# defuse/zebra

Measured on AMD Instinct MI355X. Metric: Sapling Groth16 proofs verified/sec (batch 64k) at 1/2/4/8 MI355X, higher is better.
Workload: dtype u32

## Files before the change

zebra_amd/csrc/gen_fq29.py:

```python
#!/usr/bin/env python3
import sys

P = 0x1a0111ea397fe69a4b1ba7b6434bacd764774b84f38512bf6730d2a0f6b0f6241eabfffeb153ffffb9feffffffffaaab
D = 14
W = 29
MASK = (1 << W) - 1
P29 = [(P >> (W * i)) & MASK for i in range(D)]
PINV = (-pow(P, -1, 1 << W)) % (1 << W)
_q = [((2 * P) >> (W * i)) & MASK for i in range(D)]
P2B = [_q[i] + ((1 << W) if i < D - 1 else 0) - (1 if i > 0 else 0) for i in range(D)]
assert sum(b << (W * i) for i, b in enumerate(P2B)) == 2 * P and all(b >= MASK for b in P2B[:D - 1])
assert P2B[D - 1] >= (P >> (W * (D - 1)))


KP_MAX = 12


def borrowed(k):
    q = [((k * P) >> (W * i)) & MASK for i in range(D)]
    if k == 0:
        return q
    b = [q[i] + ((1 << W) if i < D - 1 else 0) - (1 if i > 0 else 0) for i in range(D)]
    assert sum(x << (W * i) for i, x in enumerate(b)) == k * P and all(x >= MASK for x in b[:D - 1])
    if k >= 2:
        assert ((k - 1) * P) >> (W * (D - 1)) <= b[D - 1], k
    return b


def split(dst, src):
    out = []
    for L in range(D):
        b = W * L
        w, o = b >> 5, b & 31
        if o + W <= 32:
            e = "%s[%d]" % (src, w) if o == 0 else "(%s[%d] >> %d)" % (src, w, o)
            if o + W < 32:
                e = "%s & FQ29_MASK" % e
        elif w + 1 < 12:
            e = "zg_alignbit(%s[%d], %s[%d], %d) & FQ29_MASK" % (src, w + 1, src, w, o)
        else:
            e = "%s[%d] >> %d" % (src, w, o)
            out.append("  %s[%d] = %s;" % (dst, L, e))
            out.append("  zg_opaque(%s[%d]);  // narrow top digit: see gen_mont29" % (dst, L))
            continue
        out.append("  %s[%d] = %s;" % (dst, L, e))
    return out


def terms(a, b, k, step=1):
    return [(a, i, b, k - i) for i in range(D) if 0 <= k - i < D]


def sq_terms(a, a2, k):
    t = [(a2, i, a, k - i) for i in range(D) if i < k - i < D]
    if k % 2 == 0 and k // 2 < D:
        t.append((a, k // 2, a, k // 2))
    return t


def redc(chains, canon=True):
    out = []
    for (r, a, _) in chains:
        out.append("  uint32_t %s_m[14], %s_u[14];" % (a, a))
        out.append("  uint64_t %s = 0;" % a)
    for k in range(2 * D - 1):
        cols = [(r, a, f(k)) for (r, a, f) in chains]
        n = max(len(t) for _, _, t in cols)
        for q in range(n):
            for (r, a, t) in cols:
                if q < len(t):
                    x, i, y, j = t[q]
                    out.append("  %s += (uint64_t)%s[%d] * %s[%d];" % (a, x, i, y, j))
        for j in range(D):
            if j < k and k - j < D:
                for (r, a, _) in cols:
                    out.append("  %s += (uint64_t)%s_m[%d] * 0x%08xu;" % (a, a, j, P29[k - j]))
        for (r, a, _) in cols:
            if k < D - 1:
                out.append("  %s_m[%d] = ((uint32_t)%s * 0x%08xu) & FQ29_MASK;" % (a, k, a, PINV))
            elif k == D - 1:
                out.append("  %s_m[%d] = ((uint32_t)%s * 0x%08xu) & 127u;" % (a, k, a, PINV))
                out.append("  zg_opaque(%s_m[%d]);" % (a, k))
        for (r, a, _) in cols:
            if k <= D - 1:
                out.append("  %s += (uint64_t)%s_m[%d] * 0x%08xu;" % (a, a, k, P29[0]))
            if k >= D - 1:
                out.append("  %s_u[%d] = (uint32_t)%s & FQ29_MASK;" % (a, k - (D - 1), a))
            out.append("  %s >>= 29;" % a)
    for (r, a, _) in chains:
        for w in range(12):
            b = 7 + 32 * w
            L, o = b // W, b % W
            parts = ["(%s_u[%d] >> %d)" % (a, L, o) if o else "%s_u[%d]" % (a, L),
                     "(%s_u[%d] << %d)" % (a, L + 1, W - o)]
            if o + 32 > 2 * W:
                parts.append("(%s_u[%d] << %d)" % (a, L + 2, 2 * W - o))
            tgt = "%s_t[%d]" % (a, w) if canon else "%s[%d]" % (r, w)
            if w == 0 and canon:
                out.append("  uint32_t %s_t[12];" % a)
            out.append("  %s = %s;" % (tgt, " | ".join(parts)))
        if canon:
            out.append("  fq29_canon(%s, %s_t);" % (r, a))
    return out


def redc_full(chains):
    out = []
    for (r, a, _) in chains:
        out.append("  uint32_t %s_m[14];" % a)
        out.append("  uint64_t %s = 0;" % a)
    for k in range(2 * D - 1):
        cols = [(r, a, f(k)) for (r, a, f) in chains]
        n = max(len(t) for _, _, t in cols)
        for q in range(n):
            for (r, a, t) in cols:
                if q < len(t):
                    x, i, y, j = t[q]
                    out.append("  %s += (uint64_t)%s[%d] * %s[%d];" % (a, x, i, y, j))
        for j in range(D):
            if j < k and k - j < D:
                for (r, a, _) in cols:
                    out.append("  %s += (uint64_t)%s_m[%d] * 0x%08xu;" % (a, a, j, P29[k - j]))
        for (r, a, _) in cols:
            if k < D:
                out.append("  %s_m[%d] = ((uint32_t)%s * 0x%08xu) & FQ29_MASK;" % (a, k, a, PINV))
                out.append("  %s += (uint64_t)%s_m[%d] * 0x%08xu;" % (a, a, k, P29[0]))
            else:
                out.append("  %s[%d] = (uint32_t)%s & FQ29_MASK;" % (r, k - D, a))
            out.append("  %s >>= 29;" % a)
    for (r, a, _) in chains:
        out.append("  %s[13] = (uint32_t)%s;" % (r, a))
    return out


def gen_mont29(name, M, NW, mname, doc_bound):
    Dm = -(-32 * NW // W)
    last = 32 * NW - W * (Dm - 1)
    Md = [(M >> (W * i)) & MASK for i in range(Dm)]
    pinv = (-pow(M, -1, 1 << W)) % (1 << W)
    assert 2 * Dm * (1 << 58) < 1 << 64
    out = ["  uint32_t A[%d], B[%d], m[%d], u[%d], t[%d];" % (Dm, Dm, Dm, Dm + 1, NW), "  uint64_t acc = 0;"]
    for L in range(Dm):
        b_ = W * L
        w, o_ = b_ >> 5, b_ & 31
        for (X, src) in (("A", "a"), ("B", "b")):
            if o_ + W <= 32:
                e = "%s[%d]" % (src, w) if o_ == 0 else "(%s[%d] >> %d)" % (src, w, o_)
                if o_ + W < 32:
                    e += " & FQ29_MASK"
            elif w + 1 < NW:
                e = "zg_alignbit(%s[%d], %s[%d], %d) & FQ29_MASK" % (src, w + 1, src, w, o_)
            else:
                e = "%s[%d] >> %d" % (src, w, o_)
            out.append("  %s[%d] = %s;" % (X, L, e))
    out.append("  zg_opaque(A[%d]); zg_opaque(B[%d]);" % (Dm - 1, Dm - 1))
    for k in range(2 * Dm - 1):
        for i in range(Dm):
            if 0 <= k - i < Dm:
                out.append("  acc += (uint64_t)A[%d] * B[%d];" % (i, k - i))
        for j in range(Dm):
            if j < k and k - j < Dm:
                out.append("  acc += (uint64_t)m[%d] * 0x%08xu;" % (j, Md[k - j]))
        if k < Dm - 1:
            out.append("  m[%d] = ((uint32_t)acc * 0x%08xu) & FQ29_MASK;" % (k, pinv))
        elif k == Dm - 1:
            out.append("  m[%d] = ((uint32_t)acc * 0x%08xu) & 0x%08xu;" % (k, pinv, (1 << last) - 1))
            out.append("  zg_opaque(m[%d]);" % k)
        if k <= Dm - 1:
            out.append("  acc += (uint64_t)m[%d] * 0x%08xu;" % (k, Md[0]))
        if k >= Dm - 1:
            out.append("  u[%d] = (uint32_t)acc & FQ29_MASK;" % (k - (Dm - 1)))
        out.append("  acc >>= 29;")
    out.append("  u[%d] = (uint32_t)acc;  // u = t 2^%d < 2M 2^%d needs a digit more" % (Dm, last, last))
    for w in range(NW):
        b_ = last + 32 * w
        L, o_ = b_ // W, b_ % W
        parts = ["(u[%d] >> %d)" % (L, o_) if o_ else "u[%d]" % L]
        if L + 1 <= Dm:
            parts.append("(u[%d] << %d)" % (L + 1, W - o_))
        if o_ + 32 > 2 * W and L + 2 <= Dm:
            parts.append("(u[%d] << %d)" % (L + 2, 2 * W - o_))
        out.append("  t[%d] = %s;" % (w, " | ".join(parts)))
    out += ["#if defined(__HIP_DEVICE_COMPILE__)",
            "  uint32_t pm[%d];" % NW,
            "#pragma unroll",
            "  for (int i = 0; i < %d; i++) pm[i] = %s[i];" % (NW, mname),
            "  mp_reduce_once<%d>(r, t, pm);" % NW,
            "#else",
            "  uint32_t d[%d];" % NW, "  uint64_t bo = 0;",
            "  for (int i = 0; i < %d; i++) {" % NW,
            "    const uint64_t x = (uint64_t)t[i] - %s[i] - bo;" % mname,
            "    d[i] = (uint32_t)x;", "    bo = (x >> 63) & 1;", "  }",
            "  for (int i = 0; i < %d; i++) r[i] = bo ? t[i] : d[i];" % NW,
            "#endif"]
    return fn(name, "uint32_t* r, const uint32_t* a, const uint32_t* b", out,
              ["r = a b 2^-%d mod %s in 29-bit digits (%d digits, mixed radix: %d x 29 + %d): %s" % (
                  32 * NW, mname, Dm, Dm - 1, last, doc_bound)])


def fn(name, args, body, doc):
    return ["// " + d for d in doc] + ["ZG_INL void %s(%s) {" % (name, args)] + body + ["}", ""]


def main():
    o = ["// GENERATED by zebra_amd/csrc/gen_fq29.py -- do not edit.", "#pragma once", "namespace zg {", ""]
    o.append("static constexpr uint32_t FQ29_MASK = 0x%08xu;" % MASK)
    o.append("static constexpr uint32_t FQ_2P_B29[14] = {%s};  // 2p, digits 0..12 >= 2^29 - 1" %
             ", ".join("0x%08xu" % x for x in P2B))
    o.append("")
    o += ["ZG_INL uint32_t zg_alignbit(uint32_t hi, uint32_t lo, int s) {",
          "#if defined(__HIP_DEVICE_COMPILE__)",
          "  return __builtin_amdgcn_alignbit(hi, lo, s);",
          "#else",
          "  return (uint32_t)((((uint64_t)hi << 32) | lo) >> s);",
          "#endif",
          "}", ""]
    o += ["// an optimisation barrier: the compiler forgets what it knows about x's range (no instruction)",
          "ZG_INL void zg_opaque(uint32_t& x) {",
          "#if defined(__HIP_DEVICE_COMPILE__)",
          '  asm volatile("" : "+v"(x));',
          "#else",
          "  (void)x;",
          "#endif",
          "}", ""]
    o += ["// r = t >= p ? t - p : t  (t < 2p)",
          "ZG_INL void fq29_canon(uint32_t* r, const uint32_t* t) {",
          "#if defined(__HIP_DEVICE_COMPILE__)",
          "  uint32_t pm[12];",
          "#pragma unroll",
          "  for (int i = 0; i < 12; i++) pm[i] = FQ_P[i];",
          "  mp_reduce_once<12>(r, t, pm);",
          "#else",
          "  uint32_t d[12];",
          "  uint64_t bo = 0;",
          "  for (int i = 0; i < 12; i++) {",
          "    const uint64_t x = (uint64_t)t[i] - FQ_P[i] - bo;",
          "    d[i] = (uint32_t)x;",
          "    bo = (x >> 63) & 1;",
          "  }",
          "  for (int i = 0; i < 12; i++) r[i] = bo ? t[i] : d[i];",
          "#endif",
          "}", ""]

    body = ["  uint32_t A[14], B[14];"] + split("A", "a") + split("B", "b")
    body += redc([("r", "acc", lambda k: terms("A", "B", k))])
    o += fn("fq29_mul", "uint32_t* r, const uint32_t* a, const uint32_t* b", body,
            ["r = a b 2^-384 mod p; a b < 2^384 p (e.g. a < 4p, b < 2p) -> r < p.",
             "Column bound: 14 a*b + 14 m*p terms < 2^58 each."])
    body = ["  uint32_t A[14], A2[14];"] + split("A", "a") + ["  A2[%d] = A[%d] << 1;" % (i, i) for i in range(D)]
    body += redc([("r", "acc", lambda k: sq_terms("A", "A2", k))])
    o += fn("fq29_sqr", "uint32_t* r, const uint32_t* a", body,
            ["r = a^2 2^-384 mod p for a < 2p (a^2 < 2^384 p) -> r < p: 105 digit products, the",
             "off-diagonal ones once with a doubled operand (< 2^59: 7 + 14 terms per column, fine)."])
    body = ["  uint32_t X0[14], X1[14], Y0[14], Y1[14], N1[14];"] + split("X0", "x0") + split("X1", "x1") + \
        split("Y0", "y0") + split("Y1", "y1") + ["  N1[%d] = 0x%08xu - Y1[%d];" % (i, P2B[i], i) for i in range(D)]
    body += redc([("c0", "a0", lambda k: terms("X0", "Y0", k) + terms("X1", "N1", k)),
                  ("c1", "a1", lambda k: terms("X0", "Y1", k) + terms("X1", "Y0", k))])
    o += fn("f2_mul29", "uint32_t* c0, uint32_t* c1, const uint32_t* x0, const uint32_t* x1, const uint32_t* y0, "
            "const uint32_t* y1", body,
            ["Fq2 product, schoolbook in 29-bit digits with two reductions:",
             "  c0 = REDC(x0 y0 + x1 (2p - y1)),  c1 = REDC(x0 y1 + x1 y0)",
             "x lazy (< 2p per coefficient), y canonical: c0's sum < 2p p + 2p 2p = 6p^2 < 2^384 p, so both",
             "results are < p after the conditional subtraction (the contract of f2_mul_kind). Column bound",
             "for c0: 14 terms < 2^58, 14 terms < 2^59 (2p - y1 digits < 2^30), 14 m*p terms: < 2^64."])
    body = ["  uint32_t X0[14], X1[14], S[14];"] + split("X0", "x0") + split("X1", "x1") + split("S", "s")
    body += redc([("c0", "a0", lambda k: terms("X0", "S", k)), ("c1", "a1", lambda k: terms("X1", "S", k))])
    o += fn("f2_mul_fq29", "uint32_t* c0, uint32_t* c1, const uint32_t* x0, const uint32_t* x1, const uint32_t* s",
            body, ["(x0 s, x1 s) for x lazy (< 2p), s canonical -> canonical"])
    body = ["  uint32_t X0[14], X1[14], D[14], S[14], T[14];"] + split("X0", "x0") + split("X1", "x1") + \
        split("D", "dif") + ["  S[%d] = X0[%d] + X1[%d];\n  T[%d] = X1[%d] << 1;" % (i, i, i, i, i) for i in range(D)]
    body += redc([("c0", "a0", lambda k: terms("S", "D", k)), ("c1", "a1", lambda k: terms("X0", "T", k))])
    o += fn("f2_sqr29", "uint32_t* c0, uint32_t* c1, const uint32_t* x0, const uint32_t* x1, const uint32_t* dif",
            body, ["x^2 for canonical x given dif = x0 - x1 mod p: c0 = (x0 + x1) dif, c1 = x0 (2 x1). The sum and",
                   "the doubled digits are formed digit-wise (< 2^30). Column bound: 14 terms < 2^59 + 14 m*p."])
    RP = 2 ** (D * W)
    kin = (2 ** (2 * D * W - 384)) % P
    kout = (2 ** 384) % P
    o.append("static constexpr uint32_t FQ29D_KIN[14] = {%s};  // 2^428 mod p: R -> R' = 2^406" %
             ", ".join("0x%08xu" % ((kin >> (W * i)) & MASK) for i in range(D)))
    o.append("static constexpr uint32_t FQ29D_KOUT[14] = {%s};  // 2^384 mod p: R' -> R" %
             ", ".join("0x%08xu" % ((kout >> (W * i)) & MASK) for i in range(D)))
    o.append("")
    body = redc_full([("r", "acc", lambda k: terms("a", "b", k))])
    o += fn("fq29d_mul", "uint32_t* r, const uint32_t* a, const uint32_t* b", body,
            ["r = a b 2^-406 mod p in digits: a, b < 2p (normalized digits) -> r < 2p (normalized).",
             "r may alias neither a nor b."])
    body = ["  uint32_t A2[14];"] + ["  A2[%d] = a[%d] << 1;" % (i, i) for i in range(D)]
    body += redc_full([("r", "acc", lambda k: sq_terms("a", "A2", k))])
    o += fn("fq29d_sqr", "uint32_t* r, const uint32_t* a", body,
            ["r = a^2 2^-406 mod p in digits (a < 2p) -> r < 2p; r may not alias a."])
    body = ["  uint32_t A[14];"] + split("A", "a")
    body += redc_full([("r", "acc", lambda k: terms("A", "FQ29D_KIN", k))])
    o += fn("fq29d_from_mont", "uint32_t* r, const uint32_t* a",
            body, ["12-word a R (any a < 2^384) -> 14-digit a R' (< 2p)"])
    body = ["  uint32_t u[14], t[12];"] + redc_full([("u", "acc", lambda k: terms("a", "FQ29D_KOUT", k))])
    for w in range(12):
        b_ = 32 * w
        L, o_ = b_ // W, b_ % W
        parts = ["(u[%d] >> %d)" % (L, o_) if o_ else "u[%d]" % L, "(u[%d] << %d)" % (L + 1, W - o_)]
        if o_ + 32 > 2 * W:
            parts.append("(u[%d] << %d)" % (L + 2, 2 * W - o_))
        body.append("  t[%d] = %s;" % (w, " | ".join(parts)))
    body.append("  fq29_canon(r, t);")
    o += fn("fq29d_to_mont", "uint32_t* r, const uint32_t* a", body,
            ["14-digit a R' (< 2p) -> canonical 12-word a R"])

    body = redc_full([("r0", "a0", lambda k: terms("a", "b", k)), ("r1", "a1", lambda k: terms("c", "d", k))])
    o += fn("fq29d_mul2", "uint32_t* r0, uint32_t* r1, const uint32_t* a, const uint32_t* b, const uint32_t* c, "
            "const uint32_t* d", body,
            ["r0 = a b 2^-406, r1 = c d 2^-406 mod p in digits, the two chains interleaved (an Fq2 square as",
             "(x0 + x1)(x0 - x1), x0 (2 x1); an Fq2 times an Fq). Digit bounds: max(a) max(b) < 3.5 2^58, same",
             "for c d (one operand may hold unnormalized digits < 2^30). Outputs normalized, < a b / 2^406 + p."])
    body = redc_full([("c0", "a0", lambda k: terms("x0", "y0", k) + terms("x1", "n1", k)),
                      ("c1", "a1", lambda k: terms("x0", "y1", k) + terms("x1", "y0", k))])
    o += fn("f2d_mul29", "uint32_t* c0, uint32_t* c1, const uint32_t* x0, const uint32_t* x1, const uint32_t* y0, "
            "const uint32_t* y1, const uint32_t* n1", body,
            ["Fq2 product in digits, schoolbook with two reductions (the MAC structure of f2_mul29):",
             "  c0 = REDC'(x0 y0 + x1 n1),  c1 = REDC'(x0 y1 + x1 y0),  n1 = k p - y1 digit-wise (>= 0).",
             "x, y normalized (digits < 2^29), n1 digits < 2^30: 14 (2^58 + 2^59) + 14 2^58 < 2^64."])
    body = ["  uint32_t t[12];"]
    for w in range(12):
        b_ = 32 * w
        L, o_ = b_ // W, b_ % W
        parts = ["(u[%d] >> %d)" % (L, o_) if o_ else "u[%d]" % L, "(u[%d] << %d)" % (L + 1, W - o_)]
        if o_ + 32 > 2 * W:
            parts.append("(u[%d] << %d)" % (L + 2, 2 * W - o_))
        body.append("  t[%d] = %s;" % (w, " | ".join(parts)))
    body.append("  fq29_canon(r, t);")
    o += fn("fq29d_pack", "uint32_t* r, const uint32_t* u", body,
            ["14 normalized digits of a value < 2p -> its canonical 12 words (the repack and conditional",
             "subtraction that close fq29_mul)"])
    for (nm, sh, doc) in (("fq29d_split", 0, "12 words -> 14 digits of the same value"),
                          ("fq29d_split22", 22, "12 words a -> 14 digits of 2^22 a (a R -> a R' = 2^406, "
                                                "unreduced: < 2^22 p for canonical a)")):
        body = []
        for L in range(D):
            s_ = W * L - sh
            if s_ < 0:
                body.append("  d[%d] = (a[0] << %d) & FQ29_MASK;" % (L, -s_))
                continue
            w, o_ = s_ >> 5, s_ & 31
            if o_ + W <= 32:
                e = "a[%d]" % w if o_ == 0 else "(a[%d] >> %d)" % (w, o_)
                if o_ + W < 32:
                    e += " & FQ29_MASK"
            elif w + 1 < 12:
                e = "zg_alignbit(a[%d], a[%d], %d) & FQ29_MASK" % (w + 1, w, o_)
            else:
                e = "a[%d] >> %d" % (w, o_)
            body.append("  d[%d] = %s;" % (L, e))
            if w + 1 >= 12 and o_ + W > 32:
                body.append("  zg_opaque(d[%d]);  // narrow top digit: see gen_mont29" % L)
        o += fn(nm, "uint32_t* d, const uint32_t* a", body, [doc])
    pinv22 = PINV & ((1 << 22) - 1)
    assert (P * pinv22 + 1) % (1 << 22) == 0
    body = ["  uint32_t u[14], t[12];", "  uint32_t m = (a[0] * 0x%08xu) & 0x3fffffu;" % pinv22, "  zg_opaque(m);",
            "  uint64_t acc = 0;"]
    for k in range(D):
        body.append("  acc += a[%d];" % k)
        body.append("  acc += (uint64_t)m * 0x%08xu;" % P29[k])
        body.append("  u[%d] = (uint32_t)acc%s;" % (k, " & FQ29_MASK" if k < D - 1 else ""))
        if k < D - 1:
            body.append("  acc >>= 29;")
    for w in range(12):
        b_ = 22 + 32 * w
        L, o_ = b_ // W, b_ % W
        parts = ["(u[%d] >> %d)" % (L, o_) if o_ else "u[%d]" % L, "(u[%d] << %d)" % (L + 1, W - o_)]
        if o_ + 32 > 2 * W and L + 2 < D:
            parts.append("(u[%d] << %d)" % (L + 2, 2 * W - o_))
        body.append("  t[%d] = %s;" % (w, " | ".join(parts)))
    body.append("  fq29_canon(r, t);")
    o += fn("fq29d_red22", "uint32_t* r, const uint32_t* a", body,
            ["14-digit a R' (normalized, any value < 2^22 p) -> canonical 12-word a R: (a + m p) / 2^22 with",
             "m = -a / p mod 2^22, < 2p before the conditional subtraction"])

    R_BLS = 0x73eda753299d7d483339d80809a1d80553bda402fffe5bfeffffffff00000001
    P_BN = 0x30644e72e131a029b85045b68181585d97816a916871ca8d3c208c16d87cfd47
    o += gen_mont29("fr29_mul", R_BLS, 8, "FR_R", "a, b < r -> r' < r")
    o += gen_mont29("bq29_mul", P_BN, 8, "BQ_P", "a, b < p -> r < p")

    o.append("#define ZG_KP_MAX %d" % KP_MAX)
    o.append("// k p (12 words) and k p with borrowed 29-bit digits (digits 0..12 >= 2^29 - 1, top digit")
    o.append("// >= the top digit of any y <= (k - 1) p), k = 0..%d" % KP_MAX)
    o.append("static constexpr uint32_t FQ_KP[%d][12] = {%s};" % (KP_MAX + 1, ", ".join(
        "{%s}" % ", ".join("0x%08xu" % ((k * P >> (32 * i)) & 0xffffffff) for i in range(12)) for k in range(KP_MAX + 1))))
    o.append("static constexpr uint32_t FQ_KP_B29[%d][14] = {%s};" % (KP_MAX + 1, ", ".join(
        "{%s}" % ", ".join("0x%08xu" % x for x in borrowed(k)) for k in range(KP_MAX + 1))))
    o.append("")
    body = ["  uint32_t X0[14], X1[14], Y0[14], Y1[14], N1[14];"] + split("X0", "x0") + split("X1", "x1") + \
        split("Y0", "y0") + split("Y1", "y1") + ["  N1[%d] = off[%d] - Y1[%d];" % (i, i, i) for i in range(D)]
    body += redc([("c0", "a0", lambda k: terms("X0", "Y0", k) + terms("X1", "N1", k)),
                  ("c1", "a1", lambda k: terms("X0", "Y1", k) + terms("X1", "Y0", k))], canon=False)
    o += fn("f2_mul29_raw", "uint32_t* c0, uint32_t* c1, const uint32_t* x0, const uint32_t* x1, const uint32_t* y0, "
            "const uint32_t* y1, const uint32_t* off", body,
            ["f2_mul29 with y1 <= (k - 1) p and off = FQ_KP_B29[k]: c0 = REDC(x0 y0 + x1 (k p - y1)),",
             "c1 = REDC(x0 y1 + x1 y0), unreduced (< S / 2^384 + p). x, y < 2^384 (digits < 2^29)."])
    body = ["  uint32_t X0[14], X1[14], S[14];"] + split("X0", "x0") + split("X1", "x1") + split("S", "s")
    body += redc([("c0", "a0", lambda k: terms("X0", "S", k)), ("c1", "a1", lambda k: terms("X1", "S", k))],
                 canon=False)
    o += fn("f2_mul_fq29_raw", "uint32_t* c0, uint32_t* c1, const uint32_t* x0, const uint32_t* x1, const uint32_t* s",
            body, ["(x0 s, x1 s), unreduced"])
    body = ["  uint32_t X0[14], X1[14], D[14], S[14], T[14];"] + split("X0", "x0") + split("X1", "x1") + \
        split("D", "dif") + ["  S[%d] = X0[%d] + X1[%d];\n  T[%d] = X1[%d] << 1;" % (i, i, i, i, i) for i in range(D)]
    body += redc([("c0", "a0", lambda k: terms("S", "D", k)), ("c1", "a1", lambda k: terms("X0", "T", k))],
                 canon=False)
    o += fn("f2_sqr29_raw", "uint32_t* c0, uint32_t* c1, const uint32_t* x0, const uint32_t* x1, const uint32_t* dif",
            body, ["x^2 with dif = x0 - x1 + k p (any x < 2^384): c0 = (x0 + x1) dif, c1 = x0 (2 x1), unreduced"])
    o.append("}  // namespace zg")
    sys.stdout.write("\n".join(o) + "\n")


if __name__ == "__main__":
    main()
```

zebra_amd/csrc/zg_decode.h:

```cpp
#pragma once
#include "zg_batch.h"

namespace zg {

#ifndef ZG_DECODE_FQD
#define ZG_DECODE_FQD 1
#endif
#if ZG_DECODE_FQD
#define ZG_DEC_SUBGROUP g1_in_subgroup_d
#ifndef ZG_DEC_GLV
#define ZG_DEC_GLV g1_glv_mul_d
#endif
#else
#define ZG_DEC_SUBGROUP g1_in_subgroup
#define ZG_DEC_GLV g1_glv_mul
#endif

#if defined(ZG_TU_DECODE_SQRT)
#ifndef ZG_DECODE_SQRT_WPE
#define ZG_DECODE_SQRT_WPE ZG_DECODE_WPE
#endif
__global__ void __launch_bounds__(64, ZG_DECODE_SQRT_WPE) k_decode_sqrt(BatchBufs b) {
  const int role = blockIdx.x & 1;
  const int i = (blockIdx.x >> 1) * 64 + (threadIdx.x & 63);
  if (blockIdx.x == 0 && threadIdx.x < 2) b.bfail[threadIdx.x] = 0;
  if (i >= b.npad) return;
  G1A p;
  p.inf = true;
  if (i < b.n && g1_decompress(b.proofs + (size_t)i * 192 + (role == 0 ? 0 : 144), &p, false) != DEC_OK)
    p.inf = true;
  b.ptAC[(size_t)role * b.npad + i] = p;
}
#else

#if ZG_DECODE_FQD
struct GlvTabLds {
  uint32_t* base;
  __device__ __forceinline__ void put(int e, int c, const FqD& v) const {
#pragma unroll
    for (int d = 0; d < 14; d++) base[((e * 2 + c) * 14 + d) * 64] = v.d[d];
  }
  __device__ __forceinline__ FqD get(int e, int c) const {
    FqD v;
#pragma unroll
    for (int d = 0; d < 14; d++) v.d[d] = base[((e * 2 + c) * 14 + d) * 64];
    return v;
  }
};
__global__ void __launch_bounds__(64, ZG_DECODE_WPE) k_decode_glv_lds(BatchBufs b) {
  __shared__ uint32_t lds_tab[8 * 2 * 14 * 64];
  const int i = blockIdx.x * 64 + (threadIdx.x & 63);
  if (i >= b.npad) return;
  const G1A p = b.ptAC[i];
  G1A o;
  o.inf = true;
  if (!p.inf) {
    uint64_t ra, rb;
    batch_scalar_ab(b.r + (size_t)i * 16, &ra, &rb);
    const GlvTabLds tab{lds_tab + (threadIdx.x & 63)};
    G1J j;
    g1_glv_mul_w2_t(&j, &p, ra, rb, tab);
    o = jac_to_aff(j);
  }
  b.ptA[i] = o;
}
#endif

template <int JOB>
__global__ void __launch_bounds__(64, ZG_DECODE_WPE) k_decode_points(BatchBufs b, int cglv) {
  const int G = (b.npad + 63) / 64, nglv = cglv ? 2 * G : G;
  const int blk = JOB == -2 ? nglv + (int)blockIdx.x : JOB <= 0 ? (int)blockIdx.x : JOB == 1 ? nglv + (int)blockIdx.x
                                                                                     : nglv + 2 * G + (int)blockIdx.x;
  const int job = JOB >= 0 ? JOB : blk < nglv ? 0 : blk < nglv + 2 * G ? 1 : 2;
  const int role = job == 0 ? (blk < G ? 0 : 1) : job == 2 ? 2 : ((blk - nglv) & 1);
  const int grp = job == 0 ? (blk < G ? blk : blk - G) : job == 2 ? blk - nglv - 2 * G : (blk - nglv) >> 1;
  const int i = grp * 64 + (threadIdx.x & 63);
  if (i >= b.npad) return;
  if (job == 2) {
    G2A q;
    q.inf = true;
    bool ok = false;
    if (i < b.n) ok = g2_decompress(b.proofs + (size_t)i * 192 + 48, &q, false) == DEC_OK;
    b.ptB[i] = q;
    b.okbits[3 * i + 2] = ok;
    return;
  }
  const G1A p = b.ptAC[(size_t)role * b.npad + i];
  const bool ok = !p.inf;
  if (job == 1) {
    b.okbits[3 * i + role] = ok && ZG_DEC_SUBGROUP(p);
    return;
  }
  uint64_t ra = 0, rb = 0;
  if (ok) batch_scalar_ab(b.r + (size_t)i * 16, &ra, &rb);
  if (role == 1) {
    const int kind = i < b.n ? b.kinds[i] : 0;
    const G1J o = ok ? ZG_DEC_GLV(p, ra, rb) : jac_infinity<Fq>();
    for (int k = 0; k < ZG_NKINDS; k++) b.ctree[((size_t)b.npad + i) * ZG_NKINDS + k] = k == kind ? o : jac_infinity<Fq>();
    return;
  }
  G1A o;
  o.inf = true;
  if (ok) o = jac_to_aff(ZG_DEC_GLV(p, ra, rb));
  b.ptA[i] = o;
}

__global__ void __launch_bounds__(64) k_decode_finish(BatchBufs b) {
  const int i = blockIdx.x * 64 + (threadIdx.x & 63);
  if (i >= b.npad) return;
  const bool live = i < b.n;
  const int leaf = b.npad + i;
  const int kind = live ? b.kinds[i] : 0;
  uint8_t st = ST_PENDING;
  int k = 0, kk = 0;
  const uint8_t* in = b.inputs + (size_t)i * 288;
  if (live) {
    k = b.ninputs ? b.ninputs[i] : KIND_NINPUTS[kind];
    kk = k < ZG_MAX_INPUTS ? k : ZG_MAX_INPUTS;
    const bool ok = b.okbits[3 * i] && b.okbits[3 * i + 1] && b.okbits[3 * i + 2];
    bool canon = true;
#pragma unroll
    for (int j = 0; j < ZG_MAX_INPUTS; j++)
      if (j < kk) canon = canon && fp_lt_modulus<FrM>(fr_limbs_from_le(in + 32 * j));
    if (!canon)
      st = ST_INPUT_NONCANONICAL;
    else if (!ok)
      st = ST_DECODE_INVALID;
    else if (k + 1 != b.vks[kind].ic_len)
      st = ST_MALFORMED_VK;
    b.status[i] = st;
  }
  const bool pend = live && st == ST_PENDING;
  if (!pend) b.ptA[i].inf = true;
  if (!pend)
    for (int kd = 0; kd < ZG_NKINDS; kd++) b.ctree[(size_t)leaf * ZG_NKINDS + kd] = jac_infinity<Fq>();
  b.ptB[i].inf = !(live && (st == ST_PENDING || st == ST_MALFORMED_VK));
  for (int kd = 0; kd < ZG_NKINDS; kd++) {
    Fr* s = b.stree + (leaf * ZG_NKINDS + kd) * ZG_MAX_IC;
    for (int m = 0; m < ZG_MAX_IC; m++) s[m] = fp_zero<FrM>();
  }
  if (pend) {
    uint64_t ra, rb;
    batch_scalar_ab(b.r + (size_t)i * 16, &ra, &rb);
    const Fr rf = batch_scalar_fr(ra, rb);
    Fr* s = b.stree + (leaf * ZG_NKINDS + kind) * ZG_MAX_IC;
    s[0] = rf;
#pragma unroll
    for (int j = 0; j < ZG_MAX_INPUTS; j++)
      if (j < kk) s[1 + j] = fr_mul(rf, fr_to_mont(fr_limbs_from_le(in + 32 * j)));
  }
}

#endif

}
```

zebra_amd/csrc/zg_fq29_gen.h:

```cpp
#pragma once
namespace zg {

static constexpr uint32_t FQ29_MASK = 0x1fffffffu;
static constexpr uint32_t FQ_2P_B29[14] = {0x3fff5556u, 0x3feffffeu, 0x29ffffdbu, 0x2ffffac4u, 0x3ec483d4u, 0x32a0f6afu, 0x35fb3985u, 0x213ce143u, 0x2ec8ee96u, 0x2434baccu, 0x258dd3dau, 0x25ff9a68u, 0x20223d46u, 0x00000019u};

ZG_INL uint32_t zg_alignbit(uint32_t hi, uint32_t lo, int s) {
#if defined(__HIP_DEVICE_COMPILE__)
  return __builtin_amdgcn_alignbit(hi, lo, s);
#else
  return (uint32_t)((((uint64_t)hi << 32) | lo) >> s);
#endif
}

ZG_INL void zg_opaque(uint32_t& x) {
#if defined(__HIP_DEVICE_COMPILE__)
  asm volatile("" : "+v"(x));
#else
  (void)x;
#endif
}

ZG_INL void fq29_canon(uint32_t* r, const uint32_t* t) {
#if defined(__HIP_DEVICE_COMPILE__)
  uint32_t pm[12];
// ... 4821 lines not shown
  acc += (uint64_t)acc_m[0] * 0x0afd9cc3u;
  acc += (uint64_t)acc_m[1] * 0x09507b58u;
  acc += (uint64_t)acc_m[2] * 0x0f6241eau;
  acc += (uint64_t)acc_m[3] * 0x17fffd62u;
  acc += (uint64_t)acc_m[4] * 0x14ffffeeu;
  acc += (uint64_t)acc_m[5] * 0x0ff7ffffu;
  acc_m[6] = ((uint32_t)acc * 0x1ffcfffdu) & FQ29_MASK;
  acc += (uint64_t)acc_m[6] * 0x1fffaaabu;
  acc >>= 29;
  acc += (uint64_t)A2[0] * a[7];
  acc += (uint64_t)A2[1] * a[6];
  acc += (uint64_t)A2[2] * a[5];
  acc += (uint64_t)A2[3] * a[4];
  acc += (uint64_t)acc_m[0] * 0x109e70a2u;
  acc += (uint64_t)acc_m[1] * 0x0afd9cc3u;
  acc += (uint64_t)acc_m[2] * 0x09507b58u;
  acc += (uint64_t)acc_m[3] * 0x0f6241eau;
  acc += (uint64_t)acc_m[4] * 0x17fffd62u;
  acc += (uint64_t)acc_m[5] * 0x14ffffeeu;
  acc += (uint64_t)acc_m[6] * 0x0ff7ffffu;
  acc_m[7] = ((uint32_t)acc * 0x1ffcfffdu) & FQ29_MASK;
  acc += (uint64_t)acc_m[7] * 0x1fffaaabu;
  acc >>= 29;
  acc += (uint64_t)A2[0] * a[8];
  acc += (uint64_t)A2[1] * a[7];
  acc += (uint64_t)A2[2] * a[6];
  acc += (uint64_t)A2[3] * a[5];
  acc += (uint64_t)a[4] * a[4];
  acc += (uint64_t)acc_m[0] * 0x1764774bu;
  acc += (uint64_t)acc_m[1] * 0x109e70a2u;
  acc += (uint64_t)acc_m[2] * 0x0afd9cc3u;
  acc += (uint64_t)acc_m[3] * 0x09507b58u;
  acc += (uint64_t)acc_m[4] * 0x0f6241eau;
  acc += (uint64_t)acc_m[5] * 0x17fffd62u;
  acc += (uint64_t)acc_m[6] * 0x14ffffeeu;
  acc += (uint64_t)acc_m[7] * 0x0ff7ffffu;
  acc_m[8] = ((uint32_t)acc * 0x1ffcfffdu) & FQ29_MASK;
  acc += (uint64_t)acc_m[8] * 0x1fffaaabu;
  acc >>= 29;
  acc += (uint64_t)A2[0] * a[9];
  acc += (uint64_t)A2[1] * a[8];
  acc += (uint64_t)A2[2] * a[7];
  acc += (uint64_t)A2[3] * a[6];
  acc += (uint64_t)A2[4] * a[5];
  acc += (uint64_t)acc_m[0] * 0x121a5d66u;
  acc += (uint64_t)acc_m[1] * 0x1764774bu;
  acc += (uint64_t)acc_m[2] * 0x109e70a2u;
  acc += (uint64_t)acc_m[3] * 0x0afd9cc3u;
  acc += (uint64_t)acc_m[4] * 0x09507b58u;
  acc += (uint64_t)acc_m[5] * 0x0f6241eau;
  acc += (uint64_t)acc_m[6] * 0x17fffd62u;
  acc += (uint64_t)acc_m[7] * 0x14ffffeeu;
  acc += (uint64_t)acc_m[8] * 0x0ff7ffffu;
  acc_m[9] = ((uint32_t)acc * 0x1ffcfffdu) & FQ29_MASK;
  acc += (uint64_t)acc_m[9] * 0x1fffaaabu;
  acc >>= 29;
  acc += (uint64_t)A2[0] * a[10];
  acc += (uint64_t)A2[1] * a[9];
  acc += (uint64_t)A2[2] * a[8];
  acc += (uint64_t)A2[3] * a[7];
  acc += (uint64_t)A2[4] * a[6];
  acc += (uint64_t)a[5] * a[5];
  acc += (uint64_t)acc_m[0] * 0x12c6e9edu;
  acc += (uint64_t)acc_m[1] * 0x121a5d66u;
  acc += (uint64_t)acc_m[2] * 0x1764774bu;
  acc += (uint64_t)acc_m[3] * 0x109e70a2u;
  acc += (uint64_t)acc_m[4] * 0x0afd9cc3u;
  acc += (uint64_t)acc_m[5] * 0x09507b58u;
  acc += (uint64_t)acc_m[6] * 0x0f6241eau;
  acc += (uint64_t)acc_m[7] * 0x17fffd62u;
  acc += (uint64_t)acc_m[8] * 0x14ffffeeu;
  acc += (uint64_t)acc_m[9] * 0x0ff7ffffu;
  acc_m[10] = ((uint32_t)acc * 0x1ffcfffdu) & FQ29_MASK;
  acc += (uint64_t)acc_m[10] * 0x1fffaaabu;
  acc >>= 29;
  acc += (uint64_t)A2[0] * a[11];
  acc += (uint64_t)A2[1] * a[10];
  acc += (uint64_t)A2[2] * a[9];
  acc += (uint64_t)A2[3] * a[8];
  acc += (uint64_t)A2[4] * a[7];
  acc += (uint64_t)A2[5] * a[6];
  acc += (uint64_t)acc_m[0] * 0x12ffcd34u;
  acc += (uint64_t)acc_m[1] * 0x12c6e9edu;
  acc += (uint64_t)acc_m[2] * 0x121a5d66u;
  acc += (uint64_t)acc_m[3] * 0x1764774bu;
  acc += (uint64_t)acc_m[4] * 0x109e70a2u;
  acc += (uint64_t)acc_m[5] * 0x0afd9cc3u;
  acc += (uint64_t)acc_m[6] * 0x09507b58u;
  acc += (uint64_t)acc_m[7] * 0x0f6241eau;
  acc += (uint64_t)acc_m[8] * 0x17fffd62u;
  acc += (uint64_t)acc_m[9] * 0x14ffffeeu;
  acc += (uint64_t)acc_m[10] * 0x0ff7ffffu;
  acc_m[11] = ((uint32_t)acc * 0x1ffcfffdu) & FQ29_MASK;
  acc += (uint64_t)acc_m[11] * 0x1fffaaabu;
  acc >>= 29;
  acc += (uint64_t)A2[0] * a[12];
  acc += (uint64_t)A2[1] * a[11];
  acc += (uint64_t)A2[2] * a[10];
  acc += (uint64_t)A2[3] * a[9];
  acc += (uint64_t)A2[4] * a[8];
  acc += (uint64_t)A2[5] * a[7];
  acc += (uint64_t)a[6] * a[6];
  acc += (uint64_t)acc_m[0] * 0x00111ea3u;
  acc += (uint64_t)acc_m[1] * 0x12ffcd34u;
  acc += (uint64_t)acc_m[2] * 0x12c6e9edu;
  acc += (uint64_t)acc_m[3] * 0x121a5d66u;
  acc += (uint64_t)acc_m[4] * 0x1764774bu;
  acc += (uint64_t)acc_m[5] * 0x109e70a2u;
  acc += (uint64_t)acc_m[6] * 0x0afd9cc3u;
  acc += (uint64_t)acc_m[7] * 0x09507b58u;
  acc += (uint64_t)acc_m[8] * 0x0f6241eau;
  acc += (uint64_t)acc_m[9] * 0x17fffd62u;
  acc += (uint64_t)acc_m[10] * 0x14ffffeeu;
  acc += (uint64_t)acc_m[11] * 0x0ff7ffffu;
  acc_m[12] = ((uint32_t)acc * 0x1ffcfffdu) & FQ29_MASK;
  acc += (uint64_t)acc_m[12] * 0x1fffaaabu;
  acc >>= 29;
  acc += (uint64_t)A2[0] * a[13];
  acc += (uint64_t)A2[1] * a[12];
  acc += (uint64_t)A2[2] * a[11];
  acc += (uint64_t)A2[3] * a[10];
  acc += (uint64_t)A2[4] * a[9];
  acc += (uint64_t)A2[5] * a[8];
  acc += (uint64_t)A2[6] * a[7];
  acc += (uint64_t)acc_m[0] * 0x0000000du;
  acc += (uint64_t)acc_m[1] * 0x00111ea3u;
  acc += (uint64_t)acc_m[2] * 0x12ffcd34u;
  acc += (uint64_t)acc_m[3] * 0x12c6e9edu;
  acc += (uint64_t)acc_m[4] * 0x121a5d66u;
  acc += (uint64_t)acc_m[5] * 0x1764774bu;
  acc += (uint64_t)acc_m[6] * 0x109e70a2u;
  acc += (uint64_t)acc_m[7] * 0x0afd9cc3u;
  acc += (uint64_t)acc_m[8] * 0x09507b58u;
  acc += (uint64_t)acc_m[9] * 0x0f6241eau;
  acc += (uint64_t)acc_m[10] * 0x17fffd62u;
  acc += (uint64_t)acc_m[11] * 0x14ffffeeu;
  acc += (uint64_t)acc_m[12] * 0x0ff7ffffu;
  acc_m[13] = ((uint32_t)acc * 0x1ffcfffdu) & FQ29_MASK;
  acc += (uint64_t)acc_m[13] * 0x1fffaaabu;
  acc >>= 29;
  acc += (uint64_t)A2[1] * a[13];
  acc += (uint64_t)A2[2] * a[12];
  acc += (uint64_t)A2[3] * a[11];
  acc += (uint64_t)A2[4] * a[10];
  acc += (uint64_t)A2[5] * a[9];
  acc += (uint64_t)A2[6] * a[8];
  acc += (uint64_t)a[7] * a[7];
  acc += (uint64_t)acc_m[1] * 0x0000000du;
  acc += (uint64_t)acc_m[2] * 0x00111ea3u;
  acc += (uint64_t)acc_m[3] * 0x12ffcd34u;
  acc += (uint64_t)acc_m[4] * 0x12c6e9edu;
  acc += (uint64_t)acc_m[5] * 0x121a5d66u;
  acc += (uint64_t)acc_m[6] * 0x1764774bu;
  acc += (uint64_t)acc_m[7] * 0x109e70a2u;
  acc += (uint64_t)acc_m[8] * 0x0afd9cc3u;
  acc += (uint64_t)acc_m[9] * 0x09507b58u;
  acc += (uint64_t)acc_m[10] * 0x0f6241eau;
  acc += (uint64_t)acc_m[11] * 0x17fffd62u;
  acc += (uint64_t)acc_m[12] * 0x14ffffeeu;
  acc += (uint64_t)acc_m[13] * 0x0ff7ffffu;
  r[0] = (uint32_t)acc & FQ29_MASK;
  acc >>= 29;
  acc += (uint64_t)A2[2] * a[13];
  acc += (uint64_t)A2[3] * a[12];
  acc += (uint64_t)A2[4] * a[11];
  acc += (uint64_t)A2[5] * a[10];
  acc += (uint64_t)A2[6] * a[9];
  acc += (uint64_t)A2[7] * a[8];
  acc += (uint64_t)acc_m[2] * 0x0000000du;
  acc += (uint64_t)acc_m[3] * 0x00111ea3u;
  acc += (uint64_t)acc_m[4] * 0x12ffcd34u;
  acc += (uint64_t)acc_m[5] * 0x12c6e9edu;
  acc += (uint64_t)acc_m[6] * 0x121a5d66u;
  acc += (uint64_t)acc_m[7] * 0x1764774bu;
  acc += (uint64_t)acc_m[8] * 0x109e70a2u;
  acc += (uint64_t)acc_m[9] * 0x0afd9cc3u;
  acc += (uint64_t)acc_m[10] * 0x09507b58u;
  acc += (uint64_t)acc_m[11] * 0x0f6241eau;
  acc += (uint64_t)acc_m[12] * 0x17fffd62u;
  acc += (uint64_t)acc_m[13] * 0x14ffffeeu;
  r[1] = (uint32_t)acc & FQ29_MASK;
  acc >>= 29;
  acc += (uint64_t)A2[3] * a[13];
  acc += (uint64_t)A2[4] * a[12];
  acc += (uint64_t)A2[5] * a[11];
  acc += (uint64_t)A2[6] * a[10];
  acc += (uint64_t)A2[7] * a[9];
  acc += (uint64_t)a[8] * a[8];
  acc += (uint64_t)acc_m[3] * 0x0000000du;
  acc += (uint64_t)acc_m[4] * 0x00111ea3u;
  acc += (uint64_t)acc_m[5] * 0x12ffcd34u;
  acc += (uint64_t)acc_m[6] * 0x12c6e9edu;
  acc += (uint64_t)acc_m[7] * 0x121a5d66u;
  acc += (uint64_t)acc_m[8] * 0x1764774bu;
  acc += (uint64_t)acc_m[9] * 0x109e70a2u;
  acc += (uint64_t)acc_m[10] * 0x0afd9cc3u;
  acc += (uint64_t)acc_m[11] * 0x09507b58u;
  acc += (uint64_t)acc_m[12] * 0x0f6241eau;
  acc += (uint64_t)acc_m[13] * 0x17fffd62u;
  r[2] = (uint32_t)acc & FQ29_MASK;
  acc >>= 29;
  acc += (uint64_t)A2[4] * a[13];
  acc += (uint64_t)A2[5] * a[12];
  acc += (uint64_t)A2[6] * a[11];
  acc += (uint64_t)A2[7] * a[10];
  acc += (uint64_t)A2[8] * a[9];
  acc += (uint64_t)acc_m[4] * 0x0000000du;
  acc += (uint64_t)acc_m[5] * 0x00111ea3u;
  acc += (uint64_t)acc_m[6] * 0x12ffcd34u;
  acc += (uint64_t)acc_m[7] * 0x12c6e9edu;
  acc += (uint64_t)acc_m[8] * 0x121a5d66u;
  acc += (uint64_t)acc_m[9] * 0x1764774bu;
  acc += (uint64_t)acc_m[10] * 0x109e70a2u;
  acc += (uint64_t)acc_m[11] * 0x0afd9cc3u;
  acc += (uint64_t)acc_m[12] * 0x09507b58u;
  acc += (uint64_t)acc_m[13] * 0x0f6241eau;
  r[3] = (uint32_t)acc & FQ29_MASK;
  acc >>= 29;
  acc += (uint64_t)A2[5] * a[13];
  acc += (uint64_t)A2[6] * a[12];
  acc += (uint64_t)A2[7] * a[11];
  acc += (uint64_t)A2[8] * a[10];
  acc += (uint64_t)a[9] * a[9];
  acc += (uint64_t)acc_m[5] * 0x0000000du;
  acc += (uint64_t)acc_m[6] * 0x00111ea3u;
  acc += (uint64_t)acc_m[7] * 0x12ffcd34u;
  acc += (uint64_t)acc_m[8] * 0x12c6e9edu;
  acc += (uint64_t)acc_m[9] * 0x121a5d66u;
  acc += (uint64_t)acc_m[10] * 0x1764774bu;
  acc += (uint64_t)acc_m[11] * 0x109e70a2u;
  acc += (uint64_t)acc_m[12] * 0x0afd9cc3u;
  acc += (uint64_t)acc_m[13] * 0x09507b58u;
  r[4] = (uint32_t)acc & FQ29_MASK;
  acc >>= 29;
  acc += (uint64_t)A2[6] * a[13];
  acc += (uint64_t)A2[7] * a[12];
  acc += (uint64_t)A2[8] * a[11];
  acc += (uint64_t)A2[9] * a[10];
  acc += (uint64_t)acc_m[6] * 0x0000000du;
  acc += (uint64_t)acc_m[7] * 0x00111ea3u;
  acc += (uint64_t)acc_m[8] * 0x12ffcd34u;
  acc += (uint64_t)acc_m[9] * 0x12c6e9edu;
  acc += (uint64_t)acc_m[10] * 0x121a5d66u;
  acc += (uint64_t)acc_m[11] * 0x1764774bu;
  acc += (uint64_t)acc_m[12] * 0x109e70a2u;
  acc += (uint64_t)acc_m[13] * 0x0afd9cc3u;
  r[5] = (uint32_t)acc & FQ29_MASK;
  acc >>= 29;
  acc += (uint64_t)A2[7] * a[13];
  acc += (uint64_t)A2[8] * a[12];
  acc += (uint64_t)A2[9] * a[11];
  acc += (uint64_t)a[10] * a[10];
  acc += (uint64_t)acc_m[7] * 0x0000000du;
  acc += (uint64_t)acc_m[8] * 0x00111ea3u;
  acc += (uint64_t)acc_m[9] * 0x12ffcd34u;
  acc += (uint64_t)acc_m[10] * 0x12c6e9edu;
  acc += (uint64_t)acc_m[11] * 0x121a5d66u;
  acc += (uint64_t)acc_m[12] * 0x1764774bu;
  acc += (uint64_t)acc_m[13] * 0x109e70a2u;
  r[6] = (uint32_t)acc & FQ29_MASK;
  acc >>= 29;
  acc += (uint64_t)A2[8] * a[13];
  acc += (uint64_t)A2[9] * a[12];
  acc += (uint64_t)A2[10] * a[11];
  acc += (uint64_t)acc_m[8] * 0x0000000du;
  acc += (uint64_t)acc_m[9] * 0x00111ea3u;
  acc += (uint64_t)acc_m[10] * 0x12ffcd34u;
  acc += (uint64_t)acc_m[11] * 0x12c6e9edu;
  acc += (uint64_t)acc_m[12] * 0x121a5d66u;
  acc += (uint64_t)acc_m[13] * 0x1764774bu;
  r[7] = (uint32_t)acc & FQ29_MASK;
  acc >>= 29;
  acc += (uint64_t)A2[9] * a[13];
  acc += (uint64_t)A2[10] * a[12];
  acc += (uint64_t)a[11] * a[11];
  acc += (uint64_t)acc_m[9] * 0x0000000du;
  acc += (uint64_t)acc_m[10] * 0x00111ea3u;
  acc += (uint64_t)acc_m[11] * 0x12ffcd34u;
  acc += (uint64_t)acc_m[12] * 0x12c6e9edu;
  acc += (uint64_t)acc_m[13] * 0x121a5d66u;
  r[8] = (uint32_t)acc & FQ29_MASK;
  acc >>= 29;
  acc += (uint64_t)A2[10] * a[13];
  acc += (uint64_t)A2[11] * a[12];
  acc += (uint64_t)acc_m[10] * 0x0000000du;
  acc += (uint64_t)acc_m[11] * 0x00111ea3u;
  acc += (uint64_t)acc_m[12] * 0x12ffcd34u;
  acc += (uint64_t)acc_m[13] * 0x12c6e9edu;
  r[9] = (uint32_t)acc & FQ29_MASK;
  acc >>= 29;
  acc += (uint64_t)A2[11] * a[13];
  acc += (uint64_t)a[12] * a[12];
  acc += (uint64_t)acc_m[11] * 0x0000000du;
  acc += (uint64_t)acc_m[12] * 0x00111ea3u;
  acc += (uint64_t)acc_m[13] * 0x12ffcd34u;
  r[10] = (uint32_t)acc & FQ29_MASK;
  acc >>= 29;
  acc += (uint64_t)A2[12] * a[13];
  acc += (uint64_t)acc_m[12] * 0x0000000du;
  acc += (uint64_t)acc_m[13] * 0x00111ea3u;
  r[11] = (uint32_t)acc & FQ29_MASK;
  acc >>= 29;
  acc += (uint64_t)a[13] * a[13];
  acc += (uint64_t)acc_m[13] * 0x0000000du;
  r[12] = (uint32_t)acc & FQ29_MASK;
  acc >>= 29;
  r[13] = (uint32_t)acc;
}

ZG_INL void fq29d_from_mont(uint32_t* r, const uint32_t* a) {
  uint32_t A[14];
  A[0] = a[0] & FQ29_MASK;
  A[1] = zg_alignbit(a[1], a[0], 29) & FQ29_MASK;
  A[2] = zg_alignbit(a[2], a[1], 26) & FQ29_MASK;
  A[3] = zg_alignbit(a[3], a[2], 23) & FQ29_MASK;
  A[4] = zg_alignbit(a[4], a[3], 20) & FQ29_MASK;
  A[5] = zg_alignbit(a[5], a[4], 17) & FQ29_MASK;
  A[6] = zg_alignbit(a[6], a[5], 14) & FQ29_MASK;
  A[7] = zg_alignbit(a[7], a[6], 11) & FQ29_MASK;
  A[8] = zg_alignbit(a[8], a[7], 8) & FQ29_MASK;
  A[9] = zg_alignbit(a[9], a[8], 5) & FQ29_MASK;
  A[10] = (a[9] >> 2) & FQ29_MASK;
  A[11] = zg_alignbit(a[10], a[9], 31) & FQ29_MASK;
  A[12] = zg_alignbit(a[11], a[10], 28) & FQ29_MASK;
  A[13] = a[11] >> 25;
  zg_opaque(A[13]);
  uint32_t acc_m[14];
  uint64_t acc = 0;
  acc += (uint64_t)A[0] * FQ29D_KIN[0];
  acc_m[0] = ((uint32_t)acc * 0x1ffcfffdu) & FQ29_MASK;
  acc += (uint64_t)acc_m[0] * 0x1fffaaabu;
  acc >>= 29;
  acc += (uint64_t)A[0] * FQ29D_KIN[1];
  acc += (uint64_t)A[1] * FQ29D_KIN[0];
  acc += (uint64_t)acc_m[0] * 0x0ff7ffffu;
  acc_m[1] = ((uint32_t)acc * 0x1ffcfffdu) & FQ29_MASK;
  acc += (uint64_t)acc_m[1] * 0x1fffaaabu;
  acc >>= 29;
  acc += (uint64_t)A[0] * FQ29D_KIN[2];
  acc += (uint64_t)A[1] * FQ29D_KIN[1];
  acc += (uint64_t)A[2] * FQ29D_KIN[0];
  acc += (uint64_t)acc_m[0] * 0x14ffffeeu;
  acc += (uint64_t)acc_m[1] * 0x0ff7ffffu;
  acc_m[2] = ((uint32_t)acc * 0x1ffcfffdu) & FQ29_MASK;
  acc += (uint64_t)acc_m[2] * 0x1fffaaabu;
  acc >>= 29;
  acc += (uint64_t)A[0] * FQ29D_KIN[3];
  acc += (uint64_t)A[1] * FQ29D_KIN[2];
  acc += (uint64_t)A[2] * FQ29D_KIN[1];
  acc += (uint64_t)A[3] * FQ29D_KIN[0];
  acc += (uint64_t)acc_m[0] * 0x17fffd62u;
  acc += (uint64_t)acc_m[1] * 0x14ffffeeu;
  acc += (uint64_t)acc_m[2] * 0x0ff7ffffu;
  acc_m[3] = ((uint32_t)acc * 0x1ffcfffdu) & FQ29_MASK;
  acc += (uint64_t)acc_m[3] * 0x1fffaaabu;
  acc >>= 29;
  acc += (uint64_t)A[0] * FQ29D_KIN[4];
  acc += (uint64_t)A[1] * FQ29D_KIN[3];
  acc += (uint64_t)A[2] * FQ29D_KIN[2];
  acc += (uint64_t)A[3] * FQ29D_KIN[1];
  acc += (uint64_t)A[4] * FQ29D_KIN[0];
  acc += (uint64_t)acc_m[0] * 0x0f6241eau;
  acc += (uint64_t)acc_m[1] * 0x17fffd62u;
  acc += (uint64_t)acc_m[2] * 0x14ffffeeu;
  acc += (uint64_t)acc_m[3] * 0x0ff7ffffu;
  acc_m[4] = ((uint32_t)acc * 0x1ffcfffdu) & FQ29_MASK;
  acc += (uint64_t)acc_m[4] * 0x1fffaaabu;
  acc >>= 29;
  acc += (uint64_t)A[0] * FQ29D_KIN[5];
  acc += (uint64_t)A[1] * FQ29D_KIN[4];
  acc += (uint64_t)A[2] * FQ29D_KIN[3];
  acc += (uint64_t)A[3] * FQ29D_KIN[2];
  acc += (uint64_t)A[4] * FQ29D_KIN[1];
  acc += (uint64_t)A[5] * FQ29D_KIN[0];
  acc += (uint64_t)acc_m[0] * 0x09507b58u;
  acc += (uint64_t)acc_m[1] * 0x0f6241eau;
  acc += (uint64_t)acc_m[2] * 0x17fffd62u;
  acc += (uint64_t)acc_m[3] * 0x14ffffeeu;
  acc += (uint64_t)acc_m[4] * 0x0ff7ffffu;
  acc_m[5] = ((uint32_t)acc * 0x1ffcfffdu) & FQ29_MASK;
  acc += (uint64_t)acc_m[5] * 0x1fffaaabu;
  acc >>= 29;
  acc += (uint64_t)A[0] * FQ29D_KIN[6];
  acc += (uint64_t)A[1] * FQ29D_KIN[5];
  acc += (uint64_t)A[2] * FQ29D_KIN[4];
  acc += (uint64_t)A[3] * FQ29D_KIN[3];
  acc += (uint64_t)A[4] * FQ29D_KIN[2];
  acc += (uint64_t)A[5] * FQ29D_KIN[1];
  acc += (uint64_t)A[6] * FQ29D_KIN[0];
  acc += (uint64_t)acc_m[0] * 0x0afd9cc3u;
  acc += (uint64_t)acc_m[1] * 0x09507b58u;
  acc += (uint64_t)acc_m[2] * 0x0f6241eau;
  acc += (uint64_t)acc_m[3] * 0x17fffd62u;
  acc += (uint64_t)acc_m[4] * 0x14ffffeeu;
  acc += (uint64_t)acc_m[5] * 0x0ff7ffffu;
  acc_m[6] = ((uint32_t)acc * 0x1ffcfffdu) & FQ29_MASK;
  acc += (uint64_t)acc_m[6] * 0x1fffaaabu;
  acc >>= 29;
  acc += (uint64_t)A[0] * FQ29D_KIN[7];
  acc += (uint64_t)A[1] * FQ29D_KIN[6];
  acc += (uint64_t)A[2] * FQ29D_KIN[5];
  acc += (uint64_t)A[3] * FQ29D_KIN[4];
  acc += (uint64_t)A[4] * FQ29D_KIN[3];
  acc += (uint64_t)A[5] * FQ29D_KIN[2];
  acc += (uint64_t)A[6] * FQ29D_KIN[1];
  acc += (uint64_t)A[7] * FQ29D_KIN[0];
  acc += (uint64_t)acc_m[0] * 0x109e70a2u;
  acc += (uint64_t)acc_m[1] * 0x0afd9cc3u;
  acc += (uint64_t)acc_m[2] * 0x09507b58u;
  acc += (uint64_t)acc_m[3] * 0x0f6241eau;
  acc += (uint64_t)acc_m[4] * 0x17fffd62u;
  acc += (uint64_t)acc_m[5] * 0x14ffffeeu;
  acc += (uint64_t)acc_m[6] * 0x0ff7ffffu;
  acc_m[7] = ((uint32_t)acc * 0x1ffcfffdu) & FQ29_MASK;
  acc += (uint64_t)acc_m[7] * 0x1fffaaabu;
  acc >>= 29;
  acc += (uint64_t)A[0] * FQ29D_KIN[8];
  acc += (uint64_t)A[1] * FQ29D_KIN[7];
  acc += (uint64_t)A[2] * FQ29D_KIN[6];
  acc += (uint64_t)A[3] * FQ29D_KIN[5];
  acc += (uint64_t)A[4] * FQ29D_KIN[4];
  acc += (uint64_t)A[5] * FQ29D_KIN[3];
  acc += (uint64_t)A[6] * FQ29D_KIN[2];
  acc += (uint64_t)A[7] * FQ29D_KIN[1];
  acc += (uint64_t)A[8] * FQ29D_KIN[0];
  acc += (uint64_t)acc_m[0] * 0x1764774bu;
  acc += (uint64_t)acc_m[1] * 0x109e70a2u;
  acc += (uint64_t)acc_m[2] * 0x0afd9cc3u;
  acc += (uint64_t)acc_m[3] * 0x09507b58u;
  acc += (uint64_t)acc_m[4] * 0x0f6241eau;
  acc += (uint64_t)acc_m[5] * 0x17fffd62u;
  acc += (uint64_t)acc_m[6] * 0x14ffffeeu;
  acc += (uint64_t)acc_m[7] * 0x0ff7ffffu;
  acc_m[8] = ((uint32_t)acc * 0x1ffcfffdu) & FQ29_MASK;
  acc += (uint64_t)acc_m[8] * 0x1fffaaabu;
  acc >>= 29;
  acc += (uint64_t)A[0] * FQ29D_KIN[9];
  acc += (uint64_t)A[1] * FQ29D_KIN[8];
  acc += (uint64_t)A[2] * FQ29D_KIN[7];
  acc += (uint64_t)A[3] * FQ29D_KIN[6];
  acc += (uint64_t)A[4] * FQ29D_KIN[5];
  acc += (uint64_t)A[5] * FQ29D_KIN[4];
  acc += (uint64_t)A[6] * FQ29D_KIN[3];
  acc += (uint64_t)A[7] * FQ29D_KIN[2];
  acc += (uint64_t)A[8] * FQ29D_KIN[1];
  acc += (uint64_t)A[9] * FQ29D_KIN[0];
  acc += (uint64_t)acc_m[0] * 0x121a5d66u;
  acc += (uint64_t)acc_m[1] * 0x1764774bu;
  acc += (uint64_t)acc_m[2] * 0x109e70a2u;
  acc += (uint64_t)acc_m[3] * 0x0afd9cc3u;
  acc += (uint64_t)acc_m[4] * 0x09507b58u;
  acc += (uint64_t)acc_m[5] * 0x0f6241eau;
  acc += (uint64_t)acc_m[6] * 0x17fffd62u;
  acc += (uint64_t)acc_m[7] * 0x14ffffeeu;
  acc += (uint64_t)acc_m[8] * 0x0ff7ffffu;
  acc_m[9] = ((uint32_t)acc * 0x1ffcfffdu) & FQ29_MASK;
  acc += (uint64_t)acc_m[9] * 0x1fffaaabu;
  acc >>= 29;
  acc += (uint64_t)A[0] * FQ29D_KIN[10];
  acc += (uint64_t)A[1] * FQ29D_KIN[9];
  acc += (uint64_t)A[2] * FQ29D_KIN[8];
  acc += (uint64_t)A[3] * FQ29D_KIN[7];
  acc += (uint64_t)A[4] * FQ29D_KIN[6];
  acc += (uint64_t)A[5] * FQ29D_KIN[5];
  acc += (uint64_t)A[6] * FQ29D_KIN[4];
  acc += (uint64_t)A[7] * FQ29D_KIN[3];
  acc += (uint64_t)A[8] * FQ29D_KIN[2];
  acc += (uint64_t)A[9] * FQ29D_KIN[1];
  acc += (uint64_t)A[10] * FQ29D_KIN[0];
  acc += (uint64_t)acc_m[0] * 0x12c6e9edu;
  acc += (uint64_t)acc_m[1] * 0x121a5d66u;
  acc += (uint64_t)acc_m[2] * 0x1764774bu;
  acc += (uint64_t)acc_m[3] * 0x109e70a2u;
  acc += (uint64_t)acc_m[4] * 0x0afd9cc3u;
  acc += (uint64_t)acc_m[5] * 0x09507b58u;
  acc += (uint64_t)acc_m[6] * 0x0f6241eau;
  acc += (uint64_t)acc_m[7] * 0x17fffd62u;
  acc += (uint64_t)acc_m[8] * 0x14ffffeeu;
  acc += (uint64_t)acc_m[9] * 0x0ff7ffffu;
  acc_m[10] = ((uint32_t)acc * 0x1ffcfffdu) & FQ29_MASK;
  acc += (uint64_t)acc_m[10] * 0x1fffaaabu;
  acc >>= 29;
  acc += (uint64_t)A[0] * FQ29D_KIN[11];
  acc += (uint64_t)A[1] * FQ29D_KIN[10];
  acc += (uint64_t)A[2] * FQ29D_KIN[9];
  acc += (uint64_t)A[3] * FQ29D_KIN[8];
  acc += (uint64_t)A[4] * FQ29D_KIN[7];
  acc += (uint64_t)A[5] * FQ29D_KIN[6];
  acc += (uint64_t)A[6] * FQ29D_KIN[5];
  acc += (uint64_t)A[7] * FQ29D_KIN[4];
  acc += (uint64_t)A[8] * FQ29D_KIN[3];
  acc += (uint64_t)A[9] * FQ29D_KIN[2];
  acc += (uint64_t)A[10] * FQ29D_KIN[1];
  acc += (uint64_t)A[11] * FQ29D_KIN[0];
  acc += (uint64_t)acc_m[0] * 0x12ffcd34u;
  acc += (uint64_t)acc_m[1] * 0x12c6e9edu;
  acc += (uint64_t)acc_m[2] * 0x121a5d66u;
  acc += (uint64_t)acc_m[3] * 0x1764774bu;
  acc += (uint64_t)acc_m[4] * 0x109e70a2u;
  acc += (uint64_t)acc_m[5] * 0x0afd9cc3u;
  acc += (uint64_t)acc_m[6] * 0x09507b58u;
  acc += (uint64_t)acc_m[7] * 0x0f6241eau;
  acc += (uint64_t)acc_m[8] * 0x17fffd62u;
  acc += (uint64_t)acc_m[9] * 0x14ffffeeu;
  acc += (uint64_t)acc_m[10] * 0x0ff7ffffu;
  acc_m[11] = ((uint32_t)acc * 0x1ffcfffdu) & FQ29_MASK;
  acc += (uint64_t)acc_m[11] * 0x1fffaaabu;
  acc >>= 29;
  acc += (uint64_t)A[0] * FQ29D_KIN[12];
  acc += (uint64_t)A[1] * FQ29D_KIN[11];
  acc += (uint64_t)A[2] * FQ29D_KIN[10];
  acc += (uint64_t)A[3] * FQ29D_KIN[9];
  acc += (uint64_t)A[4] * FQ29D_KIN[8];
  acc += (uint64_t)A[5] * FQ29D_KIN[7];
  acc += (uint64_t)A[6] * FQ29D_KIN[6];
  acc += (uint64_t)A[7] * FQ29D_KIN[5];
  acc += (uint64_t)A[8] * FQ29D_KIN[4];
  acc += (uint64_t)A[9] * FQ29D_KIN[3];
  acc += (uint64_t)A[10] * FQ29D_KIN[2];
  acc += (uint64_t)A[11] * FQ29D_KIN[1];
  acc += (uint64_t)A[12] * FQ29D_KIN[0];
  acc += (uint64_t)acc_m[0] * 0x00111ea3u;
  acc += (uint64_t)acc_m[1] * 0x12ffcd34u;
  acc += (uint64_t)acc_m[2] * 0x12c6e9edu;
  acc += (uint64_t)acc_m[3] * 0x121a5d66u;
  acc += (uint64_t)acc_m[4] * 0x1764774bu;
  acc += (uint64_t)acc_m[5] * 0x109e70a2u;
  acc += (uint64_t)acc_m[6] * 0x0afd9cc3u;
  acc += (uint64_t)acc_m[7] * 0x09507b58u;
  acc += (uint64_t)acc_m[8] * 0x0f6241eau;
  acc += (uint64_t)acc_m[9] * 0x17fffd62u;
  acc += (uint64_t)acc_m[10] * 0x14ffffeeu;
  acc += (uint64_t)acc_m[11] * 0x0ff7ffffu;
  acc_m[12] = ((uint32_t)acc * 0x1ffcfffdu) & FQ29_MASK;
  acc += (uint64_t)acc_m[12] * 0x1fffaaabu;
  acc >>= 29;
  acc += (uint64_t)A[0] * FQ29D_KIN[13];
  acc += (uint64_t)A[1] * FQ29D_KIN[12];
  acc += (uint64_t)A[2] * FQ29D_KIN[11];
  acc += (uint64_t)A[3] * FQ29D_KIN[10];
  acc += (uint64_t)A[4] * FQ29D_KIN[9];
  acc += (uint64_t)A[5] * FQ29D_KIN[8];
  acc += (uint64_t)A[6] * FQ29D_KIN[7];
  acc += (uint64_t)A[7] * FQ29D_KIN[6];
  acc += (uint64_t)A[8] * FQ29D_KIN[5];
  acc += (uint64_t)A[9] * FQ29D_KIN[4];
  acc += (uint64_t)A[10] * FQ29D_KIN[3];
  acc += (uint64_t)A[11] * FQ29D_KIN[2];
  acc += (uint64_t)A[12] * FQ29D_KIN[1];
  acc += (uint64_t)A[13] * FQ29D_KIN[0];
  acc += (uint64_t)acc_m[0] * 0x0000000du;
  acc += (uint64_t)acc_m[1] * 0x00111ea3u;
  acc += (uint64_t)acc_m[2] * 0x12ffcd34u;
  acc += (uint64_t)acc_m[3] * 0x12c6e9edu;
  acc += (uint64_t)acc_m[4] * 0x121a5d66u;
  acc += (uint64_t)acc_m[5] * 0x1764774bu;
  acc += (uint64_t)acc_m[6] * 0x109e70a2u;
  acc += (uint64_t)acc_m[7] * 0x0afd9cc3u;
  acc += (uint64_t)acc_m[8] * 0x09507b58u;
  acc += (uint64_t)acc_m[9] * 0x0f6241eau;
  acc += (uint64_t)acc_m[10] * 0x17fffd62u;
  acc += (uint64_t)acc_m[11] * 0x14ffffeeu;
  acc += (uint64_t)acc_m[12] * 0x0ff7ffffu;
  acc_m[13] = ((uint32_t)acc * 0x1ffcfffdu) & FQ29_MASK;
  acc += (uint64_t)acc_m[13] * 0x1fffaaabu;
  acc >>= 29;
  acc += (uint64_t)A[1] * FQ29D_KIN[13];
  acc += (uint64_t)A[2] * FQ29D_KIN[12];
  acc += (uint64_t)A[3] * FQ29D_KIN[11];
  acc += (uint64_t)A[4] * FQ29D_KIN[10];
  acc += (uint64_t)A[5] * FQ29D_KIN[9];
  acc += (uint64_t)A[6] * FQ29D_KIN[8];
  acc += (uint64_t)A[7] * FQ29D_KIN[7];
  acc += (uint64_t)A[8] * FQ29D_KIN[6];
  acc += (uint64_t)A[9] * FQ29D_KIN[5];
  acc += (uint64_t)A[10] * FQ29D_KIN[4];
  acc += (uint64_t)A[11] * FQ29D_KIN[3];
  acc += (uint64_t)A[12] * FQ29D_KIN[2];
  acc += (uint64_t)A[13] * FQ29D_KIN[1];
  acc += (uint64_t)acc_m[1] * 0x0000000du;
  acc += (uint64_t)acc_m[2] * 0x00111ea3u;
  acc += (uint64_t)acc_m[3] * 0x12ffcd34u;
  acc += (uint64_t)acc_m[4] * 0x12c6e9edu;
  acc += (uint64_t)acc_m[5] * 0x121a5d66u;
  acc += (uint64_t)acc_m[6] * 0x1764774bu;
  acc += (uint64_t)acc_m[7] * 0x109e70a2u;
  acc += (uint64_t)acc_m[8] * 0x0afd9cc3u;
  acc += (uint64_t)acc_m[9] * 0x09507b58u;
  acc += (uint64_t)acc_m[10] * 0x0f6241eau;
  acc += (uint64_t)acc_m[11] * 0x17fffd62u;
  acc += (uint64_t)acc_m[12] * 0x14ffffeeu;
  acc += (uint64_t)acc_m[13] * 0x0ff7ffffu;
  r[0] = (uint32_t)acc & FQ29_MASK;
  acc >>= 29;
  acc += (uint64_t)A[2] * FQ29D_KIN[13];
  acc += (uint64_t)A[3] * FQ29D_KIN[12];
  acc += (uint64_t)A[4] * FQ29D_KIN[11];
  acc += (uint64_t)A[5] * FQ29D_KIN[10];
  acc += (uint64_t)A[6] * FQ29D_KIN[9];
  acc += (uint64_t)A[7] * FQ29D_KIN[8];
  acc += (uint64_t)A[8] * FQ29D_KIN[7];
  acc += (uint64_t)A[9] * FQ29D_KIN[6];
  acc += (uint64_t)A[10] * FQ29D_KIN[5];
  acc += (uint64_t)A[11] * FQ29D_KIN[4];
  acc += (uint64_t)A[12] * FQ29D_KIN[3];
  acc += (uint64_t)A[13] * FQ29D_KIN[2];
// ... 6824 lines not shown
```

zebra_amd/csrc/zg_fqd.h:

```cpp
#pragma once
#include "zg_curve.h"

namespace zg {

struct FqD {
  uint32_t d[14];
};

struct FqDK {
  uint32_t d[14];
};
constexpr FqDK fqd_kp(uint32_t k, uint32_t s) {
  uint32_t w[13] = {};
  uint64_t c = 0;
  for (int i = 0; i < 12; i++) {
    const uint64_t m = (uint64_t)FQ_P[i] * k + c;
    w[i] = (uint32_t)m;
    c = m >> 32;
  }
  w[12] = (uint32_t)c;
  FqDK r = {};
  for (int L = 0; L < 14; L++) {
    const int bit = 29 * L, wi = bit >> 5, off = bit & 31;
    uint64_t v = (uint64_t)w[wi] >> off;
    if (wi + 1 < 13) v |= (uint64_t)w[wi + 1] << (32 - off);
    r.d[L] = L < 13 ? (uint32_t)(v & 0x1fffffffu) : (uint32_t)v;
  }
  for (int L = 0; L < 14; L++) {
    if (L < 13) r.d[L] += s << 29;
    if (L > 0) r.d[L] -= s;
  }
  return r;
}

static constexpr uint32_t FQD_ONE[14] = {0x03a9fb84u, 0x0ba00690u, 0x071288f1u, 0x0f59bcc5u, 0x126cb614u,
                                         0x0585bf36u, 0x1b85ac3du, 0x1cf856fau, 0x1891ecbdu, 0x1a7eec05u,
                                         0x155a88f0u, 0x0741ac6du, 0x1317c30fu, 0x00000009u};

ZG_INL void fqd_norm(uint32_t* d) {
#pragma unroll
  for (int i = 0; i < 13; i++) {
    d[i + 1] += d[i] >> 29;
    d[i] &= FQ29_MASK;
  }
}

ZG_INL FqD fqd_one() {
  FqD r;
#pragma unroll
  for (int i = 0; i < 14; i++) r.d[i] = FQD_ONE[i];
  return r;
}
ZG_INL FqD fqd_zero() {
  FqD r;
#pragma unroll
  for (int i = 0; i < 14; i++) r.d[i] = 0u;
  return r;
}
#ifndef ZG_FQD_CALL
#define ZG_FQD_CALL 1
#endif
#if ZG_FQD_CALL
ZG_NOINL inline u32x16 fqd_mul_v(u32x16 a, u32x16 b) {
  uint32_t x[14], y[14], r[14];
#pragma unroll
  for (int i = 0; i < 14; i++) {
    x[i] = a[i];
    y[i] = b[i];
  }
  fq29d_mul(r, x, y);
  u32x16 o;
#pragma unroll
  for (int i = 0; i < 14; i++) o[i] = r[i];
  o[14] = o[15] = 0;
  return o;
}
ZG_NOINL inline u32x16 fqd_sqr_v(u32x16 a) {
  uint32_t x[14], r[14];
#pragma unroll
  for (int i = 0; i < 14; i++) x[i] = a[i];
  fq29d_sqr(r, x);
  u32x16 o;
#pragma unroll
  for (int i = 0; i < 14; i++) o[i] = r[i];
  o[14] = o[15] = 0;
  return o;
}
ZG_INL u32x16 fqd_pack(const FqD& a) {
  u32x16 v;
#pragma unroll
  for (int i = 0; i < 14; i++) v[i] = a.d[i];
  v[14] = v[15] = 0;
  return v;
}
ZG_INL FqD fqd_unpack(const u32x16& v) {
  FqD r;
#pragma unroll
  for (int i = 0; i < 14; i++) r.d[i] = v[i];
  return r;
}
ZG_INL FqD fqd_mul(const FqD& a, const FqD& b) { return fqd_unpack(fqd_mul_v(fqd_pack(a), fqd_pack(b))); }
ZG_INL FqD fqd_sqr(const FqD& a) { return fqd_unpack(fqd_sqr_v(fqd_pack(a))); }
#else
ZG_INL FqD fqd_mul(const FqD& a, const FqD& b) {
  FqD r;
  fq29d_mul(r.d, a.d, b.d);
  return r;
}
ZG_INL FqD fqd_sqr(const FqD& a) {
  FqD r;
  fq29d_sqr(r.d, a.d);
  return r;
}
#endif
template <int C>
ZG_INL FqD fqd_smul(const FqD& a) {
  FqD r;
#pragma unroll
  for (int i = 0; i < 14; i++) r.d[i] = C * a.d[i];
  fqd_norm(r.d);
  return r;
}
ZG_INL FqD fqd_add(const FqD& a, const FqD& b) {
  FqD r;
#pragma unroll
  for (int i = 0; i < 14; i++) r.d[i] = a.d[i] + b.d[i];
  fqd_norm(r.d);
  return r;
}
template <int K, int CA, int CB>
ZG_INL FqD fqd_sub(const FqD& a, const FqD& b) {
  constexpr FqDK kp = fqd_kp(K, CB);
  static_assert(CB >= 1 && CB <= 13 && CA >= 0 && CA + CB <= 6, "digit budget");
  FqD r;
#pragma unroll
  for (int i = 0; i < 14; i++) r.d[i] = CA * a.d[i] + (kp.d[i] - CB * b.d[i]);
  fqd_norm(r.d);
  return r;
}
template <int K>
ZG_INL FqD fqd_sub2(const FqD& a, const FqD& b, const FqD& c) {
  constexpr FqDK kp = fqd_kp(K, 2);
  FqD r;
#pragma unroll
  for (int i = 0; i < 14; i++) r.d[i] = a.d[i] + (kp.d[i] - b.d[i] - c.d[i]);
  fqd_norm(r.d);
  return r;
}
ZG_INL bool fqd_is_zero2(const FqD& v) {
  constexpr FqDK p1 = fqd_kp(1, 0);
  bool z0 = true, z1 = true;
#pragma unroll
  for (int i = 0; i < 14; i++) {
    z0 = z0 && v.d[i] == 0u;
    z1 = z1 && v.d[i] == p1.d[i];
  }
  return z0 || z1;
}
ZG_INL bool fqd_is_zero4(const FqD& v) {
  constexpr FqDK p1 = fqd_kp(1, 0), p2 = fqd_kp(2, 0), p3 = fqd_kp(3, 0);
  bool z0 = true, z1 = true, z2 = true, z3 = true;
#pragma unroll
  for (int i = 0; i < 14; i++) {
    z0 = z0 && v.d[i] == 0u;
    z1 = z1 && v.d[i] == p1.d[i];
    z2 = z2 && v.d[i] == p2.d[i];
    z3 = z3 && v.d[i] == p3.d[i];
  }
  return z0 || z1 || z2 || z3;
}

ZG_INL FqD fqd_from(const Fq& a) {
  FqD r;
  fq29d_from_mont(r.d, a.l);
  return r;
}
ZG_INL Fq fqd_to(const FqD& a) {
  Fq r;
  fq29d_to_mont(r.l, a.d);
  return r;
}

#if defined(ZG_FQD_CHECK) && !defined(__HIP_DEVICE_COMPILE__)
inline int& fqd_check_fails() {
  static int n = 0;
  return n;
}
inline void fqd_check(const FqD& v, uint32_t K) {
  const FqDK kp = fqd_kp(K, 0);
  bool ok = true, lt = false;
  for (int i = 0; i < 13; i++) ok = ok && v.d[i] <= FQ29_MASK;
  for (int i = 13; i >= 0 && !lt; i--) {
    if (v.d[i] > kp.d[i]) break;
    lt = v.d[i] < kp.d[i];
  }
  if (!ok || !lt) fqd_check_fails()++;
}
#define FQD_CHK(v, K) fqd_check(v, K)
#else
#define FQD_CHK(v, K) ((void)0)
#endif

struct Fq2D {
  FqD c0, c1;
};
#define F2D_CHK(v, K) (FQD_CHK((v).c0, K), FQD_CHK((v).c1, K))

ZG_INL Fq2D f2d_one() { return {fqd_one(), fqd_zero()}; }
ZG_INL Fq2D f2d_from(const Fq2& a) { return {fqd_from(a.c0), fqd_from(a.c1)}; }
ZG_INL Fq2D f2d_add(const Fq2D& a, const Fq2D& b) { return {fqd_add(a.c0, b.c0), fqd_add(a.c1, b.c1)}; }
template <int C>
ZG_INL Fq2D f2d_smul(const Fq2D& a) {
  return {fqd_smul<C>(a.c0), fqd_smul<C>(a.c1)};
}
template <int K, int CA, int CB>
ZG_INL Fq2D f2d_sub(const Fq2D& a, const Fq2D& b) {
  return {fqd_sub<K, CA, CB>(a.c0, b.c0), fqd_sub<K, CA, CB>(a.c1, b.c1)};
}
template <int K>
ZG_INL Fq2D f2d_sub2(const Fq2D& a, const Fq2D& b, const Fq2D& c) {
  return {fqd_sub2<K>(a.c0, b.c0, c.c0), fqd_sub2<K>(a.c1, b.c1, c.c1)};
}
constexpr bool fqd_budget_ok(const FqDK& kp, uint32_t ca) {
  for (int i = 0; i < 14; i++)
    if ((uint64_t)kp.d[i] + (uint64_t)ca * FQ29_MASK + (i > 0 ? 7u : 0u) > 0xffffffffull) return false;
  return true;
}
template <int K>
ZG_INL FqD fqd_sub114(const FqD& a, const FqD& b, const FqD& c, const FqD& d) {
  constexpr FqDK kp = fqd_kp(K, 6);
  static_assert(fqd_budget_ok(kp, 1), "digit budget");
  FqD r;
#pragma unroll
  for (int i = 0; i < 14; i++) r.d[i] = a.d[i] + (kp.d[i] - b.d[i] - c.d[i] - 4u * d.d[i]);
  fqd_norm(r.d);
  return r;
}
ZG_INL Fq2D f2d_dbl_raw(const Fq2D& a) {
  Fq2D r;
#pragma unroll
  for (int i = 0; i < 14; i++) {
    r.c0.d[i] = 2u * a.c0.d[i];
    r.c1.d[i] = 2u * a.c1.d[i];
  }
  return r;
}
template <int K>
ZG_INL Fq2D f2d_negdbl_raw(const Fq2D& a) {
  constexpr FqDK kp = fqd_kp(K, 2);
  Fq2D r;
#pragma unroll
  for (int i = 0; i < 14; i++) {
    r.c0.d[i] = kp.d[i] - 2u * a.c0.d[i];
    r.c1.d[i] = kp.d[i] - 2u * a.c1.d[i];
  }
  return r;
}

template <int KY>
ZG_INL Fq2D f2d_mul(const Fq2D& x, const Fq2D& y) {
  constexpr FqDK kp = fqd_kp(KY, 1);
  uint32_t n1[14];
#pragma unroll
  for (int i = 0; i < 14; i++) n1[i] = kp.d[i] - y.c1.d[i];
  Fq2D r;
  f2d_mul29(r.c0.d, r.c1.d, x.c0.d, x.c1.d, y.c0.d, y.c1.d, n1);
  return r;
}
template <int K>
ZG_INL Fq2D f2d_sqr(const Fq2D& a) {
  const FqD dif = fqd_sub<K, 1, 1>(a.c0, a.c1);
  uint32_t s[14], t[14];
#pragma unroll
  for (int i = 0; i < 14; i++) {
    s[i] = a.c0.d[i] + a.c1.d[i];
    t[i] = a.c1.d[i] << 1;
  }
  Fq2D r;
  fq29d_mul2(r.c0.d, r.c1.d, s, dif.d, a.c0.d, t);
  return r;
}
ZG_INL Fq2D f2d_mul_w22(const Fq2D& x, const Fq2& q) {
  const Fq nq1 = fq_neg(q.c1);
  uint32_t y0[14], y1[14], n1[14];
  fq29d_split22(y0, q.c0.l);
  fq29d_split22(y1, q.c1.l);
  fq29d_split22(n1, nq1.l);
  Fq2D r;
  f2d_mul29(r.c0.d, r.c1.d, x.c0.d, x.c1.d, y0, y1, n1);
  return r;
}
ZG_INL Fq2 f2d_mul_to_w(const Fq2D& x, const Fq2& q) {
  constexpr FqDK kp = fqd_kp(2, 1);
  uint32_t y0[14], y1[14], n1[14], u0[14], u1[14];
  fq29d_split(y0, q.c0.l);
  fq29d_split(y1, q.c1.l);
#pragma unroll
  for (int i = 0; i < 14; i++) n1[i] = kp.d[i] - y1[i];
  f2d_mul29(u0, u1, x.c0.d, x.c1.d, y0, y1, n1);
  Fq2 r;
  fq29d_pack(r.c0.l, u0);
  fq29d_pack(r.c1.l, u1);
  return r;
}
ZG_INL Fq2 f2d_mulfq_to_w(const Fq2D& x, const Fq& s) {
  uint32_t sd[14], u0[14], u1[14];
  fq29d_split(sd, s.l);
  fq29d_mul2(u0, u1, x.c0.d, sd, x.c1.d, sd);
  Fq2 r;
  fq29d_pack(r.c0.l, u0);
  fq29d_pack(r.c1.l, u1);
  return r;
}
ZG_INL Fq2 f2d_to_w(const Fq2D& a) {
  Fq2 r;
  fq29d_red22(r.c0.l, a.c0.d);
  fq29d_red22(r.c1.l, a.c1.d);
  return r;
}

struct G1D {
  FqD x, y, z;
};

ZG_INL bool g1d_is_inf(const G1D& p) { return fqd_is_zero4(p.z); }
ZG_INL G1D g1d_from_aff(const FqD& x, const FqD& y) { return {x, y, fqd_one()}; }
ZG_INL G1D g1d_infinity() { return {fqd_one(), fqd_one(), fqd_zero()}; }
ZG_INL G1J g1d_to_jac(const G1D& p) { return {fqd_to(p.x), fqd_to(p.y), fqd_to(p.z)}; }

ZG_INL G1D g1d_dbl(const G1D& p) {
  const FqD A = fqd_sqr(p.x);
  const FqD B = fqd_sqr(p.y);
  const FqD C = fqd_sqr(B);
  const FqD T = fqd_sqr(fqd_add(p.x, B));
  const FqD D = fqd_smul<2>(fqd_sub2<5>(T, A, C));
  const FqD E = fqd_smul<3>(A);
  const FqD F = fqd_sqr(E);
  const FqD X3 = fqd_sub<29, 1, 2>(F, D);
  const FqD Y3a = fqd_mul(E, fqd_sub<32, 1, 1>(D, X3));
  const FqD Y3 = fqd_sub<17, 1, 1>(Y3a, fqd_smul<8>(C));
  const FqD Z3 = fqd_smul<2>(fqd_mul(p.y, p.z));
  return {X3, Y3, Z3};
}

ZG_INL FqD fqd_pick3(int k, const FqD& a, const FqD& b, const FqD& c) {
  FqD r;
#pragma unroll
  for (int i = 0; i < 14; i++) r.d[i] = k == 0 ? a.d[i] : k == 1 ? b.d[i] : c.d[i];
  return r;
}
ZG_INL void fqd_xch_put(FqD* xch, int lane, const FqD& v) {
  if (lane < 3) xch[lane] = v;
  __syncthreads();
}
ZG_INL G1D g1d_dbl_wave(const G1D& p, FqD* xch) {
  const int lane = threadIdx.x & 63, k = lane < 3 ? lane : 0;
  const FqD m1 = fqd_mul(fqd_pick3(k, p.x, p.y, p.y), fqd_pick3(k, p.x, p.y, p.z));
  fqd_xch_put(xch, lane, m1);
  const FqD A = xch[0], B = xch[1], YZ = xch[2];
  __syncthreads();
  const FqD E = fqd_smul<3>(A);
  const FqD m2 = fqd_sqr(fqd_pick3(k, B, fqd_add(p.x, B), E));
  fqd_xch_put(xch, lane, m2);
  const FqD C = xch[0], T = xch[1], F = xch[2];
  __syncthreads();
  const FqD D = fqd_smul<2>(fqd_sub2<5>(T, A, C));
  const FqD X3 = fqd_sub<29, 1, 2>(F, D);
  const FqD m3 = fqd_mul(E, fqd_sub<32, 1, 1>(D, X3));
  fqd_xch_put(xch, lane, m3);
  const FqD Y3a = xch[0];
  __syncthreads();
  const FqD Y3 = fqd_sub<17, 1, 1>(Y3a, fqd_smul<8>(C));
  const FqD Z3 = fqd_smul<2>(YZ);
  return {X3, Y3, Z3};
}

ZG_INL G1D g1d_add_aff(const G1D& p, const FqD& qx, const FqD& qy) {
  if (g1d_is_inf(p)) return g1d_from_aff(qx, qy);
  const FqD Z1Z1 = fqd_sqr(p.z);
  const FqD U2 = fqd_mul(qx, Z1Z1);
  const FqD S2 = fqd_mul(fqd_mul(qy, p.z), Z1Z1);
  const FqD H = fqd_sub<36, 1, 1>(U2, p.x);
  const FqD rr = fqd_sub<39, 2, 2>(S2, p.y);
  const FqD HH = fqd_sqr(H);
  const FqD RR = fqd_sqr(rr);
  if (fqd_is_zero2(HH)) {
    if (fqd_is_zero2(RR)) return g1d_dbl(p);
    return g1d_infinity();
  }
  const FqD I = fqd_smul<4>(HH);
  const FqD J = fqd_mul(H, I);
  const FqD V = fqd_mul(p.x, I);
  const FqD X3 = fqd_sub2<7>(RR, J, fqd_smul<2>(V));
  const FqD Y3a = fqd_mul(rr, fqd_sub<10, 1, 1>(V, X3));
  const FqD Y3 = fqd_sub<5, 1, 2>(Y3a, fqd_mul(p.y, J));
  const FqD Z3 = fqd_smul<2>(fqd_mul(p.z, H));
  return {X3, Y3, Z3};
}

ZG_INL G1D g1d_add_full(const G1D& p, const G1D& q) {
  if (g1d_is_inf(p)) return q;
  if (g1d_is_inf(q)) return p;
  const FqD Z1Z1 = fqd_sqr(p.z);
  const FqD Z2Z2 = fqd_sqr(q.z);
  const FqD U1 = fqd_mul(p.x, Z2Z2);
  const FqD U2 = fqd_mul(q.x, Z1Z1);
  const FqD S1 = fqd_mul(fqd_mul(p.y, q.z), Z2Z2);
  const FqD S2 = fqd_mul(fqd_mul(q.y, p.z), Z1Z1);
  const FqD H = fqd_sub<3, 1, 1>(U2, U1);
  const FqD rr = fqd_sub<5, 2, 2>(S2, S1);
  const FqD HH = fqd_sqr(H);
  const FqD RR = fqd_sqr(rr);
  if (fqd_is_zero2(HH)) {
    if (fqd_is_zero2(RR)) return g1d_dbl(p);
    return g1d_infinity();
  }
  const FqD I = fqd_smul<4>(HH);
  const FqD J = fqd_mul(H, I);
  const FqD V = fqd_mul(U1, I);
  const FqD X3 = fqd_sub2<7>(RR, J, fqd_smul<2>(V));
  const FqD Y3a = fqd_mul(rr, fqd_sub<10, 1, 1>(V, X3));
  const FqD Y3 = fqd_sub<5, 1, 2>(Y3a, fqd_mul(S1, J));
  const FqD Z3 = fqd_smul<2>(fqd_mul(fqd_mul(p.z, q.z), H));
  return {X3, Y3, Z3};
}

ZG_INL FqD fqd_neg2(const FqD& x) { return fqd_sub<3, 0, 1>(fqd_zero(), x); }

ZG_DEC_INL inline bool g1_in_subgroup_d(const G1A& p) {
  if (p.inf) return true;
  const FqD px = fqd_from(p.x), py = fqd_from(p.y);
  G1D q = g1d_from_aff(px, py);
  for (int i = 126; i >= 0; i--) {
    q = g1d_dbl(q);
    if ((X2_ABS[i >> 5] >> (i & 31)) & 1u) q = g1d_add_aff(q, px, py);
  }
  const G1A s = {fq_mul(p.x, fq_const(G1_BETA)), fq_neg(p.y), false};
  return jac_eq_aff(g1d_to_jac(q), s);
}

}
```

Before: 5.488 million.

## Fuse Y3 product pairs into one Montgomery dot2 reduction in G1 formulas

Adds a generated fq29d_dot2 that computes (ab + cd) with a single Montgomery reduction. It uses it for Y3 in G1 doubling, in wave doubling and in the shared add-close path, saving one reduction per point operation, and it tightens the digit-bound constants to match. It also adds an optional x^2-via-two-passes subgroup check that reuses a held addend (LDS or registers), but that path is off by default (ZG_SUBGROUP_XX=0). The trade-off is a wider per-column accumulation, which stays under 2^64 only if the operands are kept normalized.

```diff
diff --git a/zebra_amd/csrc/gen_fq29.py b/zebra_amd/csrc/gen_fq29.py
--- a/zebra_amd/csrc/gen_fq29.py
+++ b/zebra_amd/csrc/gen_fq29.py
@@ -289,6 +289,13 @@
     body += redc_full([("r", "acc", lambda k: sq_terms("a", "A2", k))])
     o += fn("fq29d_sqr", "uint32_t* r, const uint32_t* a", body,
             ["r = a^2 2^-406 mod p in digits (a < 2p) -> r < 2p; r may not alias a."])
+    body = redc_full([("r", "acc", lambda k: terms("a", "b", k) + terms("c", "d", k))])
+    o += fn("fq29d_dot2", "uint32_t* r, const uint32_t* a, const uint32_t* b, const uint32_t* c, const uint32_t* d",
+            body,
+            ["r = (a b + c d) 2^-406 mod p in digits: a sum of two products under one reduction (the c0 chain of",
+             "f2d_mul29 alone; a point formula's Y3 = rr W - Y1 (2J) as rr W + (k p - Y1)(2J)). All four operands",
+             "normalized (digits < 2^29): 14 (2^58 + 2^58) + 14 2^58 < 2^64 per column. Output normalized,",
+             "< (a b + c d) / 2^406 + p. r may alias no operand."])
     body = ["  uint32_t A[14];"] + split("A", "a")
     body += redc_full([("r", "acc", lambda k: terms("A", "FQ29D_KIN", k))])
     o += fn("fq29d_from_mont", "uint32_t* r, const uint32_t* a",
diff --git a/zebra_amd/csrc/zg_decode.h b/zebra_amd/csrc/zg_decode.h
--- a/zebra_amd/csrc/zg_decode.h
+++ b/zebra_amd/csrc/zg_decode.h
@@ -66,6 +66,22 @@
 }
 #endif
 
+#if ZG_DECODE_FQD && ZG_SUBGROUP_XX
+struct G1HoldLds {
+  uint32_t* base;
+  __device__ __forceinline__ void put(int k, const FqD& v) const {
+#pragma unroll
+    for (int d = 0; d < 14; d++) base[(k * 14 + d) * 64] = v.d[d];
+  }
+  __device__ __forceinline__ FqD get(int k) const {
+    FqD v;
+#pragma unroll
+    for (int d = 0; d < 14; d++) v.d[d] = base[(k * 14 + d) * 64];
+    return v;
+  }
+};
+#endif
+
 template <int JOB>
 __global__ void __launch_bounds__(64, ZG_DECODE_WPE) k_decode_points(BatchBufs b, int cglv) {
   const int G = (b.npad + 63) / 64, nglv = cglv ? 2 * G : G;
@@ -88,7 +104,13 @@
   const G1A p = b.ptAC[(size_t)role * b.npad + i];
   const bool ok = !p.inf;
   if (job == 1) {
+#if ZG_DECODE_FQD && ZG_SUBGROUP_XX
+    __shared__ uint32_t lds_hold[5 * 14 * 64];
+    const G1HoldLds hold{lds_hold + (threadIdx.x & 63)};
+    b.okbits[3 * i + role] = ok && g1_in_subgroup_xx(p, hold);
+#else
     b.okbits[3 * i + role] = ok && ZG_DEC_SUBGROUP(p);
+#endif
     return;
   }
   uint64_t ra = 0, rb = 0;
diff --git a/zebra_amd/csrc/zg_fq29_gen.h b/zebra_amd/csrc/zg_fq29_gen.h
--- a/zebra_amd/csrc/zg_fq29_gen.h
+++ b/zebra_amd/csrc/zg_fq29_gen.h
@@ -5147,6 +5147,654 @@
   r[11] = (uint32_t)acc & FQ29_MASK;
   acc >>= 29;
   acc += (uint64_t)a[13] * a[13];
+  acc += (uint64_t)acc_m[13] * 0x0000000du;
+  r[12] = (uint32_t)acc & FQ29_MASK;
+  acc >>= 29;
+  r[13] = (uint32_t)acc;
+}
+
+ZG_INL void fq29d_dot2(uint32_t* r, const uint32_t* a, const uint32_t* b, const uint32_t* c, const uint32_t* d) {
+  uint32_t acc_m[14];
+  uint64_t acc = 0;
+  acc += (uint64_t)a[0] * b[0];
+  acc += (uint64_t)c[0] * d[0];
+  acc_m[0] = ((uint32_t)acc * 0x1ffcfffdu) & FQ29_MASK;
+  acc += (uint64_t)acc_m[0] * 0x1fffaaabu;
+  acc >>= 29;
+  acc += (uint64_t)a[0] * b[1];
+  acc += (uint64_t)a[1] * b[0];
+  acc += (uint64_t)c[0] * d[1];
+  acc += (uint64_t)c[1] * d[0];
+  acc += (uint64_t)acc_m[0] * 0x0ff7ffffu;
+  acc_m[1] = ((uint32_t)acc * 0x1ffcfffdu) & FQ29_MASK;
+  acc += (uint64_t)acc_m[1] * 0x1fffaaabu;
+  acc >>= 29;
+  acc += (uint64_t)a[0] * b[2];
+  acc += (uint64_t)a[1] * b[1];
+  acc += (uint64_t)a[2] * b[0];
+  acc += (uint64_t)c[0] * d[2];
+  acc += (uint64_t)c[1] * d[1];
+  acc += (uint64_t)c[2] * d[0];
+  acc += (uint64_t)acc_m[0] * 0x14ffffeeu;
+  acc += (uint64_t)acc_m[1] * 0x0ff7ffffu;
+  acc_m[2] = ((uint32_t)acc * 0x1ffcfffdu) & FQ29_MASK;
+  acc += (uint64_t)acc_m[2] * 0x1fffaaabu;
+  acc >>= 29;
+  acc += (uint64_t)a[0] * b[3];
+  acc += (uint64_t)a[1] * b[2];
+  acc += (uint64_t)a[2] * b[1];
+  acc += (uint64_t)a[3] * b[0];
+  acc += (uint64_t)c[0] * d[3];
+  acc += (uint64_t)c[1] * d[2];
+  acc += (uint64_t)c[2] * d[1];
+  acc += (uint64_t)c[3] * d[0];
+  acc += (uint64_t)acc_m[0] * 0x17fffd62u;
+  acc += (uint64_t)acc_m[1] * 0x14ffffeeu;
+  acc += (uint64_t)acc_m[2] * 0x0ff7ffffu;
+  acc_m[3] = ((uint32_t)acc * 0x1ffcfffdu) & FQ29_MASK;
+  acc += (uint64_t)acc_m[3] * 0x1fffaaabu;
+  acc >>= 29;
+  acc += (uint64_t)a[0] * b[4];
+  acc += (uint64_t)a[1] * b[3];
+  acc += (uint64_t)a[2] * b[2];
+  acc += (uint64_t)a[3] * b[1];
+  acc += (uint64_t)a[4] * b[0];
+  acc += (uint64_t)c[0] * d[4];
+  acc += (uint64_t)c[1] * d[3];
+  acc += (uint64_t)c[2] * d[2];
+  acc += (uint64_t)c[3] * d[1];
+  acc += (uint64_t)c[4] * d[0];
+  acc += (uint64_t)acc_m[0] * 0x0f6241eau;
+  acc += (uint64_t)acc_m[1] * 0x17fffd62u;
+  acc += (uint64_t)acc_m[2] * 0x14ffffeeu;
+  acc += (uint64_t)acc_m[3] * 0x0ff7ffffu;
+  acc_m[4] = ((uint32_t)acc * 0x1ffcfffdu) & FQ29_MASK;
+  acc += (uint64_t)acc_m[4] * 0x1fffaaabu;
+  acc >>= 29;
+  acc += (uint64_t)a[0] * b[5];
+  acc += (uint64_t)a[1] * b[4];
+  acc += (uint64_t)a[2] * b[3];
+  acc += (uint64_t)a[3] * b[2];
+  acc += (uint64_t)a[4] * b[1];
+  acc += (uint64_t)a[5] * b[0];
+  acc += (uint64_t)c[0] * d[5];
+  acc += (uint64_t)c[1] * d[4];
+  acc += (uint64_t)c[2] * d[3];
+  acc += (uint64_t)c[3] * d[2];
+  acc += (uint64_t)c[4] * d[1];
+  acc += (uint64_t)c[5] * d[0];
+  acc += (uint64_t)acc_m[0] * 0x09507b58u;
+  acc += (uint64_t)acc_m[1] * 0x0f6241eau;
+  acc += (uint64_t)acc_m[2] * 0x17fffd62u;
+  acc += (uint64_t)acc_m[3] * 0x14ffffeeu;
+  acc += (uint64_t)acc_m[4] * 0x0ff7ffffu;
+  acc_m[5] = ((uint32_t)acc * 0x1ffcfffdu) & FQ29_MASK;
+  acc += (uint64_t)acc_m[5] * 0x1fffaaabu;
+  acc >>= 29;
+  acc += (uint64_t)a[0] * b[6];
+  acc += (uint64_t)a[1] * b[5];
+  acc += (uint64_t)a[2] * b[4];
+  acc += (uint64_t)a[3] * b[3];
+  acc += (uint64_t)a[4] * b[2];
+  acc += (uint64_t)a[5] * b[1];
+  acc += (uint64_t)a[6] * b[0];
+  acc += (uint64_t)c[0] * d[6];
+  acc += (uint64_t)c[1] * d[5];
+  acc += (uint64_t)c[2] * d[4];
+  acc += (uint64_t)c[3] * d[3];
+  acc += (uint64_t)c[4] * d[2];
+  acc += (uint64_t)c[5] * d[1];
+  acc += (uint64_t)c[6] * d[0];
+  acc += (uint64_t)acc_m[0] * 0x0afd9cc3u;
+  acc += (uint64_t)acc_m[1] * 0x09507b58u;
+  acc += (uint64_t)acc_m[2] * 0x0f6241eau;
+  acc += (uint64_t)acc_m[3] * 0x17fffd62u;
+  acc += (uint64_t)acc_m[4] * 0x14ffffeeu;
+  acc += (uint64_t)acc_m[5] * 0x0ff7ffffu;
+  acc_m[6] = ((uint32_t)acc * 0x1ffcfffdu) & FQ29_MASK;
+  acc += (uint64_t)acc_m[6] * 0x1fffaaabu;
+  acc >>= 29;
+  acc += (uint64_t)a[0] * b[7];
+  acc += (uint64_t)a[1] * b[6];
+  acc += (uint64_t)a[2] * b[5];
+  acc += (uint64_t)a[3] * b[4];
+  acc += (uint64_t)a[4] * b[3];
+  acc += (uint64_t)a[5] * b[2];
+  acc += (uint64_t)a[6] * b[1];
+  acc += (uint64_t)a[7] * b[0];
+  acc += (uint64_t)c[0] * d[7];
+  acc += (uint64_t)c[1] * d[6];
+  acc += (uint64_t)c[2] * d[5];
+  acc += (uint64_t)c[3] * d[4];
+  acc += (uint64_t)c[4] * d[3];
+  acc += (uint64_t)c[5] * d[2];
+  acc += (uint64_t)c[6] * d[1];
+  acc += (uint64_t)c[7] * d[0];
+  acc += (uint64_t)acc_m[0] * 0x109e70a2u;
+  acc += (uint64_t)acc_m[1] * 0x0afd9cc3u;
+  acc += (uint64_t)acc_m[2] * 0x09507b58u;
+  acc += (uint64_t)acc_m[3] * 0x0f6241eau;
+  acc += (uint64_t)acc_m[4] * 0x17fffd62u;
+  acc += (uint64_t)acc_m[5] * 0x14ffffeeu;
+  acc += (uint64_t)acc_m[6] * 0x0ff7ffffu;
+  acc_m[7] = ((uint32_t)acc * 0x1ffcfffdu) & FQ29_MASK;
+  acc += (uint64_t)acc_m[7] * 0x1fffaaabu;
+  acc >>= 29;
+  acc += (uint64_t)a[0] * b[8];
+  acc += (uint64_t)a[1] * b[7];
+  acc += (uint64_t)a[2] * b[6];
+  acc += (uint64_t)a[3] * b[5];
+  acc += (uint64_t)a[4] * b[4];
+  acc += (uint64_t)a[5] * b[3];
+  acc += (uint64_t)a[6] * b[2];
+  acc += (uint64_t)a[7] * b[1];
+  acc += (uint64_t)a[8] * b[0];
+  acc += (uint64_t)c[0] * d[8];
+  acc += (uint64_t)c[1] * d[7];
+  acc += (uint64_t)c[2] * d[6];
+  acc += (uint64_t)c[3] * d[5];
+  acc += (uint64_t)c[4] * d[4];
+  acc += (uint64_t)c[5] * d[3];
+  acc += (uint64_t)c[6] * d[2];
+  acc += (uint64_t)c[7] * d[1];
+  acc += (uint64_t)c[8] * d[0];
+  acc += (uint64_t)acc_m[0] * 0x1764774bu;
+  acc += (uint64_t)acc_m[1] * 0x109e70a2u;
+  acc += (uint64_t)acc_m[2] * 0x0afd9cc3u;
+  acc += (uint64_t)acc_m[3] * 0x09507b58u;
+  acc += (uint64_t)acc_m[4] * 0x0f6241eau;
+  acc += (uint64_t)acc_m[5] * 0x17fffd62u;
+  acc += (uint64_t)acc_m[6] * 0x14ffffeeu;
+  acc += (uint64_t)acc_m[7] * 0x0ff7ffffu;
+  acc_m[8] = ((uint32_t)acc * 0x1ffcfffdu) & FQ29_MASK;
+  acc += (uint64_t)acc_m[8] * 0x1fffaaabu;
+  acc >>= 29;
+  acc += (uint64_t)a[0] * b[9];
+  acc += (uint64_t)a[1] * b[8];
+  acc += (uint64_t)a[2] * b[7];
+  acc += (uint64_t)a[3] * b[6];
+  acc += (uint64_t)a[4] * b[5];
+  acc += (uint64_t)a[5] * b[4];
+  acc += (uint64_t)a[6] * b[3];
+  acc += (uint64_t)a[7] * b[2];
+  acc += (uint64_t)a[8] * b[1];
+  acc += (uint64_t)a[9] * b[0];
+  acc += (uint64_t)c[0] * d[9];
+  acc += (uint64_t)c[1] * d[8];
+  acc += (uint64_t)c[2] * d[7];
+  acc += (uint64_t)c[3] * d[6];
+  acc += (uint64_t)c[4] * d[5];
+  acc += (uint64_t)c[5] * d[4];
+  acc += (uint64_t)c[6] * d[3];
+  acc += (uint64_t)c[7] * d[2];
+  acc += (uint64_t)c[8] * d[1];
+  acc += (uint64_t)c[9] * d[0];
+  acc += (uint64_t)acc_m[0] * 0x121a5d66u;
+  acc += (uint64_t)acc_m[1] * 0x1764774bu;
+  acc += (uint64_t)acc_m[2] * 0x109e70a2u;
+  acc += (uint64_t)acc_m[3] * 0x0afd9cc3u;
+  acc += (uint64_t)acc_m[4] * 0x09507b58u;
+  acc += (uint64_t)acc_m[5] * 0x0f6241eau;
+  acc += (uint64_t)acc_m[6] * 0x17fffd62u;
+  acc += (uint64_t)acc_m[7] * 0x14ffffeeu;
+  acc += (uint64_t)acc_m[8] * 0x0ff7ffffu;
+  acc_m[9] = ((uint32_t)acc * 0x1ffcfffdu) & FQ29_MASK;
+  acc += (uint64_t)acc_m[9] * 0x1fffaaabu;
+  acc >>= 29;
+  acc += (uint64_t)a[0] * b[10];
+  acc += (uint64_t)a[1] * b[9];
+  acc += (uint64_t)a[2] * b[8];
+  acc += (uint64_t)a[3] * b[7];
+  acc += (uint64_t)a[4] * b[6];
+  acc += (uint64_t)a[5] * b[5];
+  acc += (uint64_t)a[6] * b[4];
+  acc += (uint64_t)a[7] * b[3];
+  acc += (uint64_t)a[8] * b[2];
+  acc += (uint64_t)a[9] * b[1];
+  acc += (uint64_t)a[10] * b[0];
+  acc += (uint64_t)c[0] * d[10];
+  acc += (uint64_t)c[1] * d[9];
+  acc += (uint64_t)c[2] * d[8];
+  acc += (uint64_t)c[3] * d[7];
+  acc += (uint64_t)c[4] * d[6];
+  acc += (uint64_t)c[5] * d[5];
+  acc += (uint64_t)c[6] * d[4];
+  acc += (uint64_t)c[7] * d[3];
+  acc += (uint64_t)c[8] * d[2];
+  acc += (uint64_t)c[9] * d[1];
+  acc += (uint64_t)c[10] * d[0];
+  acc += (uint64_t)acc_m[0] * 0x12c6e9edu;
+  acc += (uint64_t)acc_m[1] * 0x121a5d66u;
+  acc += (uint64_t)acc_m[2] * 0x1764774bu;
+  acc += (uint64_t)acc_m[3] * 0x109e70a2u;
+  acc += (uint64_t)acc_m[4] * 0x0afd9cc3u;
+  acc += (uint64_t)acc_m[5] * 0x09507b58u;
+  acc += (uint64_t)acc_m[6] * 0x0f6241eau;
+  acc += (uint64_t)acc_m[7] * 0x17fffd62u;
+  acc += (uint64_t)acc_m[8] * 0x14ffffeeu;
+  acc += (uint64_t)acc_m[9] * 0x0ff7ffffu;
+  acc_m[10] = ((uint32_t)acc * 0x1ffcfffdu) & FQ29_MASK;
+  acc += (uint64_t)acc_m[10] * 0x1fffaaabu;
+  acc >>= 29;
+  acc += (uint64_t)a[0] * b[11];
+  acc += (uint64_t)a[1] * b[10];
+  acc += (uint64_t)a[2] * b[9];
+  acc += (uint64_t)a[3] * b[8];
+  acc += (uint64_t)a[4] * b[7];
+  acc += (uint64_t)a[5] * b[6];
+  acc += (uint64_t)a[6] * b[5];
+  acc += (uint64_t)a[7] * b[4];
+  acc += (uint64_t)a[8] * b[3];
+  acc += (uint64_t)a[9] * b[2];
+  acc += (uint64_t)a[10] * b[1];
+  acc += (uint64_t)a[11] * b[0];
+  acc += (uint64_t)c[0] * d[11];
+  acc += (uint64_t)c[1] * d[10];
+  acc += (uint64_t)c[2] * d[9];
+  acc += (uint64_t)c[3] * d[8];
+  acc += (uint64_t)c[4] * d[7];
+  acc += (uint64_t)c[5] * d[6];
+  acc += (uint64_t)c[6] * d[5];
+  acc += (uint64_t)c[7] * d[4];
+  acc += (uint64_t)c[8] * d[3];
+  acc += (uint64_t)c[9] * d[2];
+  acc += (uint64_t)c[10] * d[1];
+  acc += (uint64_t)c[11] * d[0];
+  acc += (uint64_t)acc_m[0] * 0x12ffcd34u;
+  acc += (uint64_t)acc_m[1] * 0x12c6e9edu;
+  acc += (uint64_t)acc_m[2] * 0x121a5d66u;
+  acc += (uint64_t)acc_m[3] * 0x1764774bu;
+  acc += (uint64_t)acc_m[4] * 0x109e70a2u;
+  acc += (uint64_t)acc_m[5] * 0x0afd9cc3u;
+  acc += (uint64_t)acc_m[6] * 0x09507b58u;
+  acc += (uint64_t)acc_m[7] * 0x0f6241eau;
+  acc += (uint64_t)acc_m[8] * 0x17fffd62u;
+  acc += (uint64_t)acc_m[9] * 0x14ffffeeu;
+  acc += (uint64_t)acc_m[10] * 0x0ff7ffffu;
+  acc_m[11] = ((uint32_t)acc * 0x1ffcfffdu) & FQ29_MASK;
+  acc += (uint64_t)acc_m[11] * 0x1fffaaabu;
+  acc >>= 29;
+  acc += (uint64_t)a[0] * b[12];
+  acc += (uint64_t)a[1] * b[11];
+  acc += (uint64_t)a[2] * b[10];
+  acc += (uint64_t)a[3] * b[9];
+  acc += (uint64_t)a[4] * b[8];
+  acc += (uint64_t)a[5] * b[7];
+  acc += (uint64_t)a[6] * b[6];
+  acc += (uint64_t)a[7] * b[5];
+  acc += (uint64_t)a[8] * b[4];
+  acc += (uint64_t)a[9] * b[3];
+  acc += (uint64_t)a[10] * b[2];
+  acc += (uint64_t)a[11] * b[1];
+  acc += (uint64_t)a[12] * b[0];
+  acc += (uint64_t)c[0] * d[12];
+  acc += (uint64_t)c[1] * d[11];
+  acc += (uint64_t)c[2] * d[10];
+  acc += (uint64_t)c[3] * d[9];
+  acc += (uint64_t)c[4] * d[8];
+  acc += (uint64_t)c[5] * d[7];
+  acc += (uint64_t)c[6] * d[6];
+  acc += (uint64_t)c[7] * d[5];
+  acc += (uint64_t)c[8] * d[4];
+  acc += (uint64_t)c[9] * d[3];
+  acc += (uint64_t)c[10] * d[2];
+  acc += (uint64_t)c[11] * d[1];
+  acc += (uint64_t)c[12] * d[0];
+  acc += (uint64_t)acc_m[0] * 0x00111ea3u;
+  acc += (uint64_t)acc_m[1] * 0x12ffcd34u;
+  acc += (uint64_t)acc_m[2] * 0x12c6e9edu;
+  acc += (uint64_t)acc_m[3] * 0x121a5d66u;
+  acc += (uint64_t)acc_m[4] * 0x1764774bu;
+  acc += (uint64_t)acc_m[5] * 0x109e70a2u;
+  acc += (uint64_t)acc_m[6] * 0x0afd9cc3u;
+  acc += (uint64_t)acc_m[7] * 0x09507b58u;
+  acc += (uint64_t)acc_m[8] * 0x0f6241eau;
+  acc += (uint64_t)acc_m[9] * 0x17fffd62u;
+  acc += (uint64_t)acc_m[10] * 0x14ffffeeu;
+  acc += (uint64_t)acc_m[11] * 0x0ff7ffffu;
+  acc_m[12] = ((uint32_t)acc * 0x1ffcfffdu) & FQ29_MASK;
+  acc += (uint64_t)acc_m[12] * 0x1fffaaabu;
+  acc >>= 29;
+  acc += (uint64_t)a[0] * b[13];
+  acc += (uint64_t)a[1] * b[12];
+  acc += (uint64_t)a[2] * b[11];
+  acc += (uint64_t)a[3] * b[10];
+  acc += (uint64_t)a[4] * b[9];
+  acc += (uint64_t)a[5] * b[8];
+  acc += (uint64_t)a[6] * b[7];
+  acc += (uint64_t)a[7] * b[6];
+  acc += (uint64_t)a[8] * b[5];
+  acc += (uint64_t)a[9] * b[4];
+  acc += (uint64_t)a[10] * b[3];
+  acc += (uint64_t)a[11] * b[2];
+  acc += (uint64_t)a[12] * b[1];
+  acc += (uint64_t)a[13] * b[0];
+  acc += (uint64_t)c[0] * d[13];
+  acc += (uint64_t)c[1] * d[12];
+  acc += (uint64_t)c[2] * d[11];
+  acc += (uint64_t)c[3] * d[10];
+  acc += (uint64_t)c[4] * d[9];
+  acc += (uint64_t)c[5] * d[8];
+  acc += (uint64_t)c[6] * d[7];
+  acc += (uint64_t)c[7] * d[6];
+  acc += (uint64_t)c[8] * d[5];
+  acc += (uint64_t)c[9] * d[4];
+  acc += (uint64_t)c[10] * d[3];
+  acc += (uint64_t)c[11] * d[2];
+  acc += (uint64_t)c[12] * d[1];
+  acc += (uint64_t)c[13] * d[0];
+  acc += (uint64_t)acc_m[0] * 0x0000000du;
+  acc += (uint64_t)acc_m[1] * 0x00111ea3u;
+  acc += (uint64_t)acc_m[2] * 0x12ffcd34u;
+  acc += (uint64_t)acc_m[3] * 0x12c6e9edu;
+  acc += (uint64_t)acc_m[4] * 0x121a5d66u;
+  acc += (uint64_t)acc_m[5] * 0x1764774bu;
+  acc += (uint64_t)acc_m[6] * 0x109e70a2u;
+  acc += (uint64_t)acc_m[7] * 0x0afd9cc3u;
+  acc += (uint64_t)acc_m[8] * 0x09507b58u;
+  acc += (uint64_t)acc_m[9] * 0x0f6241eau;
+  acc += (uint64_t)acc_m[10] * 0x17fffd62u;
+  acc += (uint64_t)acc_m[11] * 0x14ffffeeu;
+  acc += (uint64_t)acc_m[12] * 0x0ff7ffffu;
+  acc_m[13] = ((uint32_t)acc * 0x1ffcfffdu) & FQ29_MASK;
+  acc += (uint64_t)acc_m[13] * 0x1fffaaabu;
+  acc >>= 29;
+  acc += (uint64_t)a[1] * b[13];
+  acc += (uint64_t)a[2] * b[12];
+  acc += (uint64_t)a[3] * b[11];
+  acc += (uint64_t)a[4] * b[10];
+  acc += (uint64_t)a[5] * b[9];
+  acc += (uint64_t)a[6] * b[8];
+  acc += (uint64_t)a[7] * b[7];
+  acc += (uint64_t)a[8] * b[6];
+  acc += (uint64_t)a[9] * b[5];
+  acc += (uint64_t)a[10] * b[4];
+  acc += (uint64_t)a[11] * b[3];
+  acc += (uint64_t)a[12] * b[2];
+  acc += (uint64_t)a[13] * b[1];
+  acc += (uint64_t)c[1] * d[13];
+  acc += (uint64_t)c[2] * d[12];
+  acc += (uint64_t)c[3] * d[11];
+  acc += (uint64_t)c[4] * d[10];
+  acc += (uint64_t)c[5] * d[9];
+  acc += (uint64_t)c[6] * d[8];
+  acc += (uint64_t)c[7] * d[7];
+  acc += (uint64_t)c[8] * d[6];
+  acc += (uint64_t)c[9] * d[5];
+  acc += (uint64_t)c[10] * d[4];
+  acc += (uint64_t)c[11] * d[3];
+  acc += (uint64_t)c[12] * d[2];
+  acc += (uint64_t)c[13] * d[1];
+  acc += (uint64_t)acc_m[1] * 0x0000000du;
+  acc += (uint64_t)acc_m[2] * 0x00111ea3u;
+  acc += (uint64_t)acc_m[3] * 0x12ffcd34u;
+  acc += (uint64_t)acc_m[4] * 0x12c6e9edu;
+  acc += (uint64_t)acc_m[5] * 0x121a5d66u;
+  acc += (uint64_t)acc_m[6] * 0x1764774bu;
+  acc += (uint64_t)acc_m[7] * 0x109e70a2u;
+  acc += (uint64_t)acc_m[8] * 0x0afd9cc3u;
+  acc += (uint64_t)acc_m[9] * 0x09507b58u;
+  acc += (uint64_t)acc_m[10] * 0x0f6241eau;
+  acc += (uint64_t)acc_m[11] * 0x17fffd62u;
+  acc += (uint64_t)acc_m[12] * 0x14ffffeeu;
+  acc += (uint64_t)acc_m[13] * 0x0ff7ffffu;
+  r[0] = (uint32_t)acc & FQ29_MASK;
+  acc >>= 29;
+  acc += (uint64_t)a[2] * b[13];
+  acc += (uint64_t)a[3] * b[12];
+  acc += (uint64_t)a[4] * b[11];
+  acc += (uint64_t)a[5] * b[10];
+  acc += (uint64_t)a[6] * b[9];
+  acc += (uint64_t)a[7] * b[8];
+  acc += (uint64_t)a[8] * b[7];
+  acc += (uint64_t)a[9] * b[6];
+  acc += (uint64_t)a[10] * b[5];
+  acc += (uint64_t)a[11] * b[4];
+  acc += (uint64_t)a[12] * b[3];
+  acc += (uint64_t)a[13] * b[2];
+  acc += (uint64_t)c[2] * d[13];
+  acc += (uint64_t)c[3] * d[12];
+  acc += (uint64_t)c[4] * d[11];
+  acc += (uint64_t)c[5] * d[10];
+  acc += (uint64_t)c[6] * d[9];
+  acc += (uint64_t)c[7] * d[8];
+  acc += (uint64_t)c[8] * d[7];
+  acc += (uint64_t)c[9] * d[6];
+  acc += (uint64_t)c[10] * d[5];
+  acc += (uint64_t)c[11] * d[4];
+  acc += (uint64_t)c[12] * d[3];
+  acc += (uint64_t)c[13] * d[2];
+  acc += (uint64_t)acc_m[2] * 0x0000000du;
+  acc += (uint64_t)acc_m[3] * 0x00111ea3u;
+  acc += (uint64_t)acc_m[4] * 0x12ffcd34u;
+  acc += (uint64_t)acc_m[5] * 0x12c6e9edu;
+  acc += (uint64_t)acc_m[6] * 0x121a5d66u;
+  acc += (uint64_t)acc_m[7] * 0x1764774bu;
+  acc += (uint64_t)acc_m[8] * 0x109e70a2u;
+  acc += (uint64_t)acc_m[9] * 0x0afd9cc3u;
+  acc += (uint64_t)acc_m[10] * 0x09507b58u;
+  acc += (uint64_t)acc_m[11] * 0x0f6241eau;
+  acc += (uint64_t)acc_m[12] * 0x17fffd62u;
+  acc += (uint64_t)acc_m[13] * 0x14ffffeeu;
+  r[1] = (uint32_t)acc & FQ29_MASK;
+  acc >>= 29;
+  acc += (uint64_t)a[3] * b[13];
+  acc += (uint64_t)a[4] * b[12];
+  acc += (uint64_t)a[5] * b[11];
+  acc += (uint64_t)a[6] * b[10];
+  acc += (uint64_t)a[7] * b[9];
+  acc += (uint64_t)a[8] * b[8];
+  acc += (uint64_t)a[9] * b[7];
+  acc += (uint64_t)a[10] * b[6];
+  acc += (uint64_t)a[11] * b[5];
+  acc += (uint64_t)a[12] * b[4];
+  acc += (uint64_t)a[13] * b[3];
+  acc += (uint64_t)c[3] * d[13];
+  acc += (uint64_t)c[4] * d[12];
+  acc += (uint64_t)c[5] * d[11];
+  acc += (uint64_t)c[6] * d[10];
+  acc += (uint64_t)c[7] * d[9];
+  acc += (uint64_t)c[8] * d[8];
+  acc += (uint64_t)c[9] * d[7];
+  acc += (uint64_t)c[10] * d[6];
+  acc += (uint64_t)c[11] * d[5];
+  acc += (uint64_t)c[12] * d[4];
+  acc += (uint64_t)c[13] * d[3];
+  acc += (uint64_t)acc_m[3] * 0x0000000du;
+  acc += (uint64_t)acc_m[4] * 0x00111ea3u;
+  acc += (uint64_t)acc_m[5] * 0x12ffcd34u;
+  acc += (uint64_t)acc_m[6] * 0x12c6e9edu;
+  acc += (uint64_t)acc_m[7] * 0x121a5d66u;
+  acc += (uint64_t)acc_m[8] * 0x1764774bu;
+  acc += (uint64_t)acc_m[9] * 0x109e70a2u;
+  acc += (uint64_t)acc_m[10] * 0x0afd9cc3u;
+  acc += (uint64_t)acc_m[11] * 0x09507b58u;
+  acc += (uint64_t)acc_m[12] * 0x0f6241eau;
+  acc += (uint64_t)acc_m[13] * 0x17fffd62u;
+  r[2] = (uint32_t)acc & FQ29_MASK;
+  acc >>= 29;
+  acc += (uint64_t)a[4] * b[13];
+  acc += (uint64_t)a[5] * b[12];
+  acc += (uint64_t)a[6] * b[11];
+  acc += (uint64_t)a[7] * b[10];
+  acc += (uint64_t)a[8] * b[9];
+  acc += (uint64_t)a[9] * b[8];
+  acc += (uint64_t)a[10] * b[7];
+  acc += (uint64_t)a[11] * b[6];
+  acc += (uint64_t)a[12] * b[5];
+  acc += (uint64_t)a[13] * b[4];
+  acc += (uint64_t)c[4] * d[13];
+  acc += (uint64_t)c[5] * d[12];
+  acc += (uint64_t)c[6] * d[11];
+  acc += (uint64_t)c[7] * d[10];
+  acc += (uint64_t)c[8] * d[9];
+  acc += (uint64_t)c[9] * d[8];
+  acc += (uint64_t)c[10] * d[7];
+  acc += (uint64_t)c[11] * d[6];
+  acc += (uint64_t)c[12] * d[5];
+  acc += (uint64_t)c[13] * d[4];
+  acc += (uint64_t)acc_m[4] * 0x0000000du;
+  acc += (uint64_t)acc_m[5] * 0x00111ea3u;
+  acc += (uint64_t)acc_m[6] * 0x12ffcd34u;
+  acc += (uint64_t)acc_m[7] * 0x12c6e9edu;
+  acc += (uint64_t)acc_m[8] * 0x121a5d66u;
+  acc += (uint64_t)acc_m[9] * 0x1764774bu;
+  acc += (uint64_t)acc_m[10] * 0x109e70a2u;
+  acc += (uint64_t)acc_m[11] * 0x0afd9cc3u;
+  acc += (uint64_t)acc_m[12] * 0x09507b58u;
+  acc += (uint64_t)acc_m[13] * 0x0f6241eau;
+  r[3] = (uint32_t)acc & FQ29_MASK;
+  acc >>= 29;
+  acc += (uint64_t)a[5] * b[13];
+  acc += (uint64_t)a[6] * b[12];
+  acc += (uint64_t)a[7] * b[11];
+  acc += (uint64_t)a[8] * b[10];
+  acc += (uint64_t)a[9] * b[9];
+  acc += (uint64_t)a[10] * b[8];
+  acc += (uint64_t)a[11] * b[7];
+  acc += (uint64_t)a[12] * b[6];
+  acc += (uint64_t)a[13] * b[5];
+  acc += (uint64_t)c[5] * d[13];
+  acc += (uint64_t)c[6] * d[12];
+  acc += (uint64_t)c[7] * d[11];
+  acc += (uint64_t)c[8] * d[10];
+  acc += (uint64_t)c[9] * d[9];
+  acc += (uint64_t)c[10] * d[8];
+  acc += (uint64_t)c[11] * d[7];
+  acc += (uint64_t)c[12] * d[6];
+  acc += (uint64_t)c[13] * d[5];
+  acc += (uint64_t)acc_m[5] * 0x0000000du;
+  acc += (uint64_t)acc_m[6] * 0x00111ea3u;
+  acc += (uint64_t)acc_m[7] * 0x12ffcd34u;
+  acc += (uint64_t)acc_m[8] * 0x12c6e9edu;
+  acc += (uint64_t)acc_m[9] * 0x121a5d66u;
+  acc += (uint64_t)acc_m[10] * 0x1764774bu;
+  acc += (uint64_t)acc_m[11] * 0x109e70a2u;
+  acc += (uint64_t)acc_m[12] * 0x0afd9cc3u;
+  acc += (uint64_t)acc_m[13] * 0x09507b58u;
+  r[4] = (uint32_t)acc & FQ29_MASK;
+  acc >>= 29;
+  acc += (uint64_t)a[6] * b[13];
+  acc += (uint64_t)a[7] * b[12];
+  acc += (uint64_t)a[8] * b[11];
+  acc += (uint64_t)a[9] * b[10];
+  acc += (uint64_t)a[10] * b[9];
+  acc += (uint64_t)a[11] * b[8];
+  acc += (uint64_t)a[12] * b[7];
+  acc += (uint64_t)a[13] * b[6];
+  acc += (uint64_t)c[6] * d[13];
+  acc += (uint64_t)c[7] * d[12];
+  acc += (uint64_t)c[8] * d[11];
+  acc += (uint64_t)c[9] * d[10];
+  acc += (uint64_t)c[10] * d[9];
+  acc += (uint64_t)c[11] * d[8];
+  acc += (uint64_t)c[12] * d[7];
+  acc += (uint64_t)c[13] * d[6];
+  acc += (uint64_t)acc_m[6] * 0x0000000du;
+  acc += (uint64_t)acc_m[7] * 0x00111ea3u;
+  acc += (uint64_t)acc_m[8] * 0x12ffcd34u;
+  acc += (uint64_t)acc_m[9] * 0x12c6e9edu;
+  acc += (uint64_t)acc_m[10] * 0x121a5d66u;
+  acc += (uint64_t)acc_m[11] * 0x1764774bu;
+  acc += (uint64_t)acc_m[12] * 0x109e70a2u;
+  acc += (uint64_t)acc_m[13] * 0x0afd9cc3u;
+  r[5] = (uint32_t)acc & FQ29_MASK;
+  acc >>= 29;
+  acc += (uint64_t)a[7] * b[13];
+  acc += (uint64_t)a[8] * b[12];
+  acc += (uint64_t)a[9] * b[11];
+  acc += (uint64_t)a[10] * b[10];
+  acc += (uint64_t)a[11] * b[9];
+  acc += (uint64_t)a[12] * b[8];
+  acc += (uint64_t)a[13] * b[7];
+  acc += (uint64_t)c[7] * d[13];
+  acc += (uint64_t)c[8] * d[12];
+  acc += (uint64_t)c[9] * d[11];
+  acc += (uint64_t)c[10] * d[10];
+  acc += (uint64_t)c[11] * d[9];
+  acc += (uint64_t)c[12] * d[8];
+  acc += (uint64_t)c[13] * d[7];
+  acc += (uint64_t)acc_m[7] * 0x0000000du;
+  acc += (uint64_t)acc_m[8] * 0x00111ea3u;
+  acc += (uint64_t)acc_m[9] * 0x12ffcd34u;
+  acc += (uint64_t)acc_m[10] * 0x12c6e9edu;
+  acc += (uint64_t)acc_m[11] * 0x121a5d66u;
+  acc += (uint64_t)acc_m[12] * 0x1764774bu;
+  acc += (uint64_t)acc_m[13] * 0x109e70a2u;
+  r[6] = (uint32_t)acc & FQ29_MASK;
+  acc >>= 29;
+  acc += (uint64_t)a[8] * b[13];
+  acc += (uint64_t)a[9] * b[12];
+  acc += (uint64_t)a[10] * b[11];
+  acc += (uint64_t)a[11] * b[10];
+  acc += (uint64_t)a[12] * b[9];
+  acc += (uint64_t)a[13] * b[8];
+  acc += (uint64_t)c[8] * d[13];
+  acc += (uint64_t)c[9] * d[12];
+  acc += (uint64_t)c[10] * d[11];
+  acc += (uint64_t)c[11] * d[10];
+  acc += (uint64_t)c[12] * d[9];
+  acc += (uint64_t)c[13] * d[8];
+  acc += (uint64_t)acc_m[8] * 0x0000000du;
+  acc += (uint64_t)acc_m[9] * 0x00111ea3u;
+  acc += (uint64_t)acc_m[10] * 0x12ffcd34u;
+  acc += (uint64_t)acc_m[11] * 0x12c6e9edu;
+  acc += (uint64_t)acc_m[12] * 0x121a5d66u;
+  acc += (uint64_t)acc_m[13] * 0x1764774bu;
+  r[7] = (uint32_t)acc & FQ29_MASK;
+  acc >>= 29;
+  acc += (uint64_t)a[9] * b[13];
+  acc += (uint64_t)a[10] * b[12];
+  acc += (uint64_t)a[11] * b[11];
+  acc += (uint64_t)a[12] * b[10];
+  acc += (uint64_t)a[13] * b[9];
+  acc += (uint64_t)c[9] * d[13];
+  acc += (uint64_t)c[10] * d[12];
+  acc += (uint64_t)c[11] * d[11];
+  acc += (uint64_t)c[12] * d[10];
+  acc += (uint64_t)c[13] * d[9];
+  acc += (uint64_t)acc_m[9] * 0x0000000du;
+  acc += (uint64_t)acc_m[10] * 0x00111ea3u;
+  acc += (uint64_t)acc_m[11] * 0x12ffcd34u;
+  acc += (uint64_t)acc_m[12] * 0x12c6e9edu;
+  acc += (uint64_t)acc_m[13] * 0x121a5d66u;
+  r[8] = (uint32_t)acc & FQ29_MASK;
+  acc >>= 29;
+  acc += (uint64_t)a[10] * b[13];
+  acc += (uint64_t)a[11] * b[12];
+  acc += (uint64_t)a[12] * b[11];
+  acc += (uint64_t)a[13] * b[10];
+  acc += (uint64_t)c[10] * d[13];
+  acc += (uint64_t)c[11] * d[12];
+  acc += (uint64_t)c[12] * d[11];
+  acc += (uint64_t)c[13] * d[10];
+  acc += (uint64_t)acc_m[10] * 0x0000000du;
+  acc += (uint64_t)acc_m[11] * 0x00111ea3u;
+  acc += (uint64_t)acc_m[12] * 0x12ffcd34u;
+  acc += (uint64_t)acc_m[13] * 0x12c6e9edu;
+  r[9] = (uint32_t)acc & FQ29_MASK;
+  acc >>= 29;
+  acc += (uint64_t)a[11] * b[13];
+  acc += (uint64_t)a[12] * b[12];
+  acc += (uint64_t)a[13] * b[11];
+  acc += (uint64_t)c[11] * d[13];
+  acc += (uint64_t)c[12] * d[12];
+  acc += (uint64_t)c[13] * d[11];
+  acc += (uint64_t)acc_m[11] * 0x0000000du;
+  acc += (uint64_t)acc_m[12] * 0x00111ea3u;
+  acc += (uint64_t)acc_m[13] * 0x12ffcd34u;
+  r[10] = (uint32_t)acc & FQ29_MASK;
+  acc >>= 29;
+  acc += (uint64_t)a[12] * b[13];
+  acc += (uint64_t)a[13] * b[12];
+  acc += (uint64_t)c[12] * d[13];
+  acc += (uint64_t)c[13] * d[12];
+  acc += (uint64_t)acc_m[12] * 0x0000000du;
+  acc += (uint64_t)acc_m[13] * 0x00111ea3u;
+  r[11] = (uint32_t)acc & FQ29_MASK;
+  acc >>= 29;
+  acc += (uint64_t)a[13] * b[13];
+  acc += (uint64_t)c[13] * d[13];
   acc += (uint64_t)acc_m[13] * 0x0000000du;
   r[12] = (uint32_t)acc & FQ29_MASK;
   acc >>= 29;
diff --git a/zebra_amd/csrc/zg_fqd.h b/zebra_amd/csrc/zg_fqd.h
--- a/zebra_amd/csrc/zg_fqd.h
+++ b/zebra_amd/csrc/zg_fqd.h
@@ -147,6 +147,12 @@
   fqd_norm(r.d);
   return r;
 }
+ZG_INL FqD fqd_neg2(const FqD& x) { return fqd_sub<3, 0, 1>(fqd_zero(), x); }
+ZG_INL FqD fqd_dot2(const FqD& a, const FqD& b, const FqD& c, const FqD& d) {
+  FqD r;
+  fq29d_dot2(r.d, a.d, b.d, c.d, d.d);
+  return r;
+}
 ZG_INL bool fqd_is_zero2(const FqD& v) {
   constexpr FqDK p1 = fqd_kp(1, 0);
   bool z0 = true, z1 = true;
@@ -319,15 +325,41 @@
   return r;
 }
 
+#ifndef ZG_G1D_DOT2
+#define ZG_G1D_DOT2 1
+#endif
+#if ZG_G1D_DOT2
+static constexpr int G1D_KX = 19, G1D_KY = 4;
+#else
+static constexpr int G1D_KX = 35, G1D_KY = 19;
+#endif
 struct G1D {
   FqD x, y, z;
 };
+#define G1D_CHK(p) (FQD_CHK((p).x, G1D_KX), FQD_CHK((p).y, G1D_KY), FQD_CHK((p).z, 4))
 
 ZG_INL bool g1d_is_inf(const G1D& p) { return fqd_is_zero4(p.z); }
 ZG_INL G1D g1d_from_aff(const FqD& x, const FqD& y) { return {x, y, fqd_one()}; }
 ZG_INL G1D g1d_infinity() { return {fqd_one(), fqd_one(), fqd_zero()}; }
 ZG_INL G1J g1d_to_jac(const G1D& p) { return {fqd_to(p.x), fqd_to(p.y), fqd_to(p.z)}; }
 
+#if ZG_G1D_DOT2
+ZG_INL G1D g1d_dbl(const G1D& p) {
+  G1D_CHK(p);
+  const FqD A = fqd_sqr(p.x);
+  const FqD B = fqd_sqr(p.y);
+  const FqD D = fqd_smul<4>(fqd_mul(p.x, B));
+  const FqD E = fqd_smul<3>(A);
+  const FqD F = fqd_sqr(E);
+  const FqD X3 = fqd_sub<17, 1, 2>(F, D);
+  const FqD W = fqd_sub<20, 1, 1>(D, X3);
+  const FqD nB = fqd_neg2(B), B8 = fqd_smul<8>(B);
+  const FqD Y3 = fqd_dot2(E, W, nB, B8);
+  const FqD Z3 = fqd_smul<2>(fqd_mul(p.y, p.z));
+  FQD_CHK(D, 8), FQD_CHK(X3, 19), FQD_CHK(W, 28), FQD_CHK(nB, 3), FQD_CHK(B8, 16), FQD_CHK(Y3, 2), FQD_CHK(Z3, 4);
+  return {X3, Y3, Z3};
+}
+#else
 ZG_INL G1D g1d_dbl(const G1D& p) {
   const FqD A = fqd_sqr(p.x);
   const FqD B = fqd_sqr(p.y);
@@ -342,6 +374,7 @@
   const FqD Z3 = fqd_smul<2>(fqd_mul(p.y, p.z));
   return {X3, Y3, Z3};
 }
+#endif
 
 ZG_INL FqD fqd_pick3(int k, const FqD& a, const FqD& b, const FqD& c) {
   FqD r;
@@ -360,6 +393,15 @@
   const FqD A = xch[0], B = xch[1], YZ = xch[2];
   __syncthreads();
   const FqD E = fqd_smul<3>(A);
+#if ZG_G1D_DOT2
+  const FqD m2 = fqd_mul(fqd_pick3(k, p.x, E, E), fqd_pick3(k, B, E, E));
+  fqd_xch_put(xch, lane, m2);
+  const FqD XB = xch[0], F = xch[1];
+  __syncthreads();
+  const FqD D = fqd_smul<4>(XB);
+  const FqD X3 = fqd_sub<17, 1, 2>(F, D);
+  const FqD Y3 = fqd_dot2(E, fqd_sub<20, 1, 1>(D, X3), fqd_neg2(B), fqd_smul<8>(B));
+#else
   const FqD m2 = fqd_sqr(fqd_pick3(k, B, fqd_add(p.x, B), E));
   fqd_xch_put(xch, lane, m2);
   const FqD C = xch[0], T = xch[1], F = xch[2];
@@ -371,19 +413,38 @@
   const FqD Y3a = xch[0];
   __syncthreads();
   const FqD Y3 = fqd_sub<17, 1, 1>(Y3a, fqd_smul<8>(C));
+#endif
   const FqD Z3 = fqd_smul<2>(YZ);
   return {X3, Y3, Z3};
 }
 
+template <int KYB>
+ZG_INL void g1d_add_close(FqD& X3, FqD& Y3, const FqD& rr, const FqD& RR, const FqD& J, const FqD& V, const FqD& Y) {
+  X3 = fqd_sub2<7>(RR, J, fqd_smul<2>(V));
+  const FqD W = fqd_sub<10, 1, 1>(V, X3);
+#if ZG_G1D_DOT2
+  const FqD nY = fqd_sub<KYB + 1, 0, 1>(fqd_zero(), Y);
+  const FqD J2 = fqd_smul<2>(J);
+  Y3 = fqd_dot2(rr, W, nY, J2);
+  FQD_CHK(nY, KYB + 1), FQD_CHK(J2, 4), FQD_CHK(Y3, 2);
+#else
+  Y3 = fqd_sub<5, 1, 2>(fqd_mul(rr, W), fqd_mul(Y, J));
+  FQD_CHK(Y3, 7);
+#endif
+  FQD_CHK(X3, 9), FQD_CHK(W, 12);
+}
+
 ZG_INL G1D g1d_add_aff(const G1D& p, const FqD& qx, const FqD& qy) {
+  G1D_CHK(p), FQD_CHK(qx, 2), FQD_CHK(qy, 4);
   if (g1d_is_inf(p)) return g1d_from_aff(qx, qy);
   const FqD Z1Z1 = fqd_sqr(p.z);
   const FqD U2 = fqd_mul(qx, Z1Z1);
   const FqD S2 = fqd_mul(fqd_mul(qy, p.z), Z1Z1);
-  const FqD H = fqd_sub<36, 1, 1>(U2, p.x);
-  const FqD rr = fqd_sub<39, 2, 2>(S2, p.y);
+  const FqD H = fqd_sub<G1D_KX + 1, 1, 1>(U2, p.x);
+  const FqD rr = fqd_sub<2 * G1D_KY + 1, 2, 2>(S2, p.y);
   const FqD HH = fqd_sqr(H);
   const FqD RR = fqd_sqr(rr);
+  FQD_CHK(H, G1D_KX + 3), FQD_CHK(rr, 2 * G1D_KY + 5);
   if (fqd_is_zero2(HH)) {
     if (fqd_is_zero2(RR)) return g1d_dbl(p);
     return g1d_infinity();
@@ -391,26 +452,27 @@
   const FqD I = fqd_smul<4>(HH);
   const FqD J = fqd_mul(H, I);
   const FqD V = fqd_mul(p.x, I);
-  const FqD X3 = fqd_sub2<7>(RR, J, fqd_smul<2>(V));
-  const FqD Y3a = fqd_mul(rr, fqd_sub<10, 1, 1>(V, X3));
-  const FqD Y3 = fqd_sub<5, 1, 2>(Y3a, fqd_mul(p.y, J));
-  const FqD Z3 = fqd_smul<2>(fqd_mul(p.z, H));
-  return {X3, Y3, Z3};
-}
-
-ZG_INL G1D g1d_add_full(const G1D& p, const G1D& q) {
-  if (g1d_is_inf(p)) return q;
-  if (g1d_is_inf(q)) return p;
+  G1D r;
+  g1d_add_close<G1D_KY>(r.x, r.y, rr, RR, J, V, p.y);
+  r.z = fqd_smul<2>(fqd_mul(p.z, H));
+  return r;
+}
+
+template <class Hold>
+ZG_INL G1D g1d_readd_t(const G1D& p, const Hold& h) {
+  G1D_CHK(p);
+  if (g1d_is_inf(p)) return {h.get(0), h.get(1), h.get(2)};
+  if (fqd_is_zero4(h.get(2))) return p;
   const FqD Z1Z1 = fqd_sqr(p.z);
-  const FqD Z2Z2 = fqd_sqr(q.z);
-  const FqD U1 = fqd_mul(p.x, Z2Z2);
-  const FqD U2 = fqd_mul(q.x, Z1Z1);
-  const FqD S1 = fqd_mul(fqd_mul(p.y, q.z), Z2Z2);
-  const FqD S2 = fqd_mul(fqd_mul(q.y, p.z), Z1Z1);
+  const FqD U1 = fqd_mul(p.x, h.get(3));
+  const FqD U2 = fqd_mul(h.get(0), Z1Z1);
+  const FqD S1 = fqd_mul(p.y, h.get(4));
+  const FqD S2 = fqd_mul(fqd_mul(h.get(1), p.z), Z1Z1);
   const FqD H = fqd_sub<3, 1, 1>(U2, U1);
   const FqD rr = fqd_sub<5, 2, 2>(S2, S1);
   const FqD HH = fqd_sqr(H);
   const FqD RR = fqd_sqr(rr);
+  FQD_CHK(H, 5), FQD_CHK(rr, 9);
   if (fqd_is_zero2(HH)) {
     if (fqd_is_zero2(RR)) return g1d_dbl(p);
     return g1d_infinity();
@@ -418,16 +480,60 @@
   const FqD I = fqd_smul<4>(HH);
   const FqD J = fqd_mul(H, I);
   const FqD V = fqd_mul(U1, I);
-  const FqD X3 = fqd_sub2<7>(RR, J, fqd_smul<2>(V));
-  const FqD Y3a = fqd_mul(rr, fqd_sub<10, 1, 1>(V, X3));
-  const FqD Y3 = fqd_sub<5, 1, 2>(Y3a, fqd_mul(S1, J));
-  const FqD Z3 = fqd_smul<2>(fqd_mul(fqd_mul(p.z, q.z), H));
-  return {X3, Y3, Z3};
-}
-
-ZG_INL FqD fqd_neg2(const FqD& x) { return fqd_sub<3, 0, 1>(fqd_zero(), x); }
-
+  G1D r;
+  g1d_add_close<2>(r.x, r.y, rr, RR, J, V, S1);
+  r.z = fqd_smul<2>(fqd_mul(fqd_mul(p.z, h.get(2)), H));
+  return r;
+}
+struct G1Hold {
+  FqD v[5];
+  ZG_HD void put(int k, const FqD& x) { v[k] = x; }
+  ZG_HD FqD get(int k) const { return v[k]; }
+};
+ZG_INL G1D g1d_readd(const G1D& p, const G1D& q, const FqD& Z2Z2, const FqD& Z2C) {
+  G1D_CHK(q), FQD_CHK(Z2Z2, 2), FQD_CHK(Z2C, 2);
+  return g1d_readd_t(p, G1Hold{{q.x, q.y, q.z, Z2Z2, Z2C}});
+}
+
+ZG_INL G1D g1d_add_full(const G1D& p, const G1D& q) {
+  if (g1d_is_inf(p)) return q;
+  if (g1d_is_inf(q)) return p;
+  const FqD Z2Z2 = fqd_sqr(q.z);
+  return g1d_readd(p, q, Z2Z2, fqd_mul(q.z, Z2Z2));
+}
+
+#ifndef ZG_SUBGROUP_XX
+#define ZG_SUBGROUP_XX 0
+#endif
+template <class Hold>
+ZG_INL bool g1_in_subgroup_xx(const G1A& p, Hold& hold) {
+  if (p.inf) return true;
+  G1D q = g1d_from_aff(fqd_from(p.x), fqd_from(p.y));
+  hold.put(0, q.x);
+  hold.put(1, q.y);
+  for (int k = 2; k < 5; k++) hold.put(k, fqd_one());
+  for (int pass = 0; pass < 2; pass++) {
+    for (int i = 62; i >= 0; i--) {
+      q = g1d_dbl(q);
+      if ((BLS_X >> i) & 1ull) q = g1d_readd_t(q, hold);
+    }
+    if (pass == 0) {
+      const FqD zz = fqd_sqr(q.z);
+      hold.put(0, q.x);
+      hold.put(1, q.y);
+      hold.put(2, q.z);
+      hold.put(3, zz);
+      hold.put(4, fqd_mul(q.z, zz));
+    }
+  }
+  const G1A s = {fq_mul(p.x, fq_const(G1_BETA)), fq_neg(p.y), false};
+  return jac_eq_aff(g1d_to_jac(q), s);
+}
 ZG_DEC_INL inline bool g1_in_subgroup_d(const G1A& p) {
+#if ZG_SUBGROUP_XX
+  G1Hold hold;
+  return g1_in_subgroup_xx(p, hold);
+#else
   if (p.inf) return true;
   const FqD px = fqd_from(p.x), py = fqd_from(p.y);
   G1D q = g1d_from_aff(px, py);
@@ -437,6 +543,7 @@
   }
   const G1A s = {fq_mul(p.x, fq_const(G1_BETA)), fq_neg(p.y), false};
   return jac_eq_aff(g1d_to_jac(q), s);
-}
-
-}
+#endif
+}
+
+}
```

After: 5.562 million (median of 6 runs). 1.4% higher.
